# MIT-SPARK/TEASER-plusplus

Hardware: AMD Instinct MI355X
Metric: registrations/sec at N=10000 correspondences, 95% outliers (higher is better)
Workload: dtype bf16x3-split MFMA + f32 filter with FP64 fix-up for K1 (bitmap bit-identical to FP64); f64 estimators

## Files before the change

include/teaser_hip.h:

```cpp
#ifndef TEASER_HIP_H_
#define TEASER_HIP_H_

#include <stddef.h>
#include <stdint.h>

#ifdef __cplusplus
extern "C" {
#endif

#define TEASER_HIP_ABI_VERSION 1

#if defined(__GNUC__)
#define TEASER_HIP_API __attribute__((visibility("default")))
#else
#define TEASER_HIP_API
#endif

typedef enum teaser_hip_status {
  TEASER_HIP_OK = 0,
  TEASER_HIP_ERR_BAD_ARG = 1,
  TEASER_HIP_ERR_HIP = 2,
  TEASER_HIP_ERR_NO_DEVICE = 3,
  TEASER_HIP_ERR_UNSUPPORTED = 4,
  TEASER_HIP_ERR_TIME_LIMIT = 5,
// ... 101 lines not shown
TEASER_HIP_API int32_t teaser_hip_multi_create(const teaser_params_c* params, const int32_t* devices,
                                int32_t n_devices , teaser_hip_multi** out);
TEASER_HIP_API int32_t teaser_hip_multi_destroy(teaser_hip_multi* mh);
TEASER_HIP_API int32_t teaser_hip_multi_solve_batch(teaser_hip_multi* mh, const double* const* src,
                                     const double* const* dst, const int32_t* n, int32_t batch,
                                     teaser_solution_c* out );
TEASER_HIP_API int32_t teaser_hip_multi_route(teaser_hip_multi* mh, int32_t problem, teaser_hip_solver** h,
                               int32_t* local_problem);
TEASER_HIP_API int32_t teaser_hip_multi_device_count(const teaser_hip_multi* mh);

#define TEASER_HIP_COMM_ID_BYTES 128
typedef struct teaser_hip_comm teaser_hip_comm;
TEASER_HIP_API int32_t teaser_hip_comm_shard(int64_t total, int32_t rank, int32_t world, int64_t* first, int64_t* last);
TEASER_HIP_API int32_t teaser_hip_comm_unique_id(uint8_t* id );
TEASER_HIP_API int32_t teaser_hip_comm_create(const uint8_t* id, int32_t rank, int32_t world, int32_t device,
                               teaser_hip_comm** out);
TEASER_HIP_API int32_t teaser_hip_comm_destroy(teaser_hip_comm* c);
TEASER_HIP_API int32_t teaser_hip_comm_gather_solutions(teaser_hip_comm* c, const teaser_solution_c* local,
                                         int64_t n_local, int64_t total, teaser_solution_c* all );
TEASER_HIP_API int32_t teaser_hip_comm_gather_indices(teaser_hip_comm* c, teaser_hip_solver* h, int64_t n_local,
                                       int64_t total, int32_t k_max, int32_t* lens, int32_t* indices);
TEASER_HIP_API const char* teaser_hip_comm_last_error(const teaser_hip_comm* c);

TEASER_HIP_API int32_t teaser_hip_get_max_clique(teaser_hip_solver* h, int32_t problem, int32_t* buf, int64_t* len);
TEASER_HIP_API int32_t teaser_hip_get_rotation_inliers(teaser_hip_solver* h, int32_t problem, int32_t* buf,
                                        int64_t* len);
TEASER_HIP_API int32_t teaser_hip_get_translation_inliers(teaser_hip_solver* h, int32_t problem, int32_t* buf,
                                           int64_t* len);
TEASER_HIP_API int32_t teaser_hip_get_input_ordered_translation_inliers(teaser_hip_solver* h, int32_t problem,
                                                         int32_t* buf, int64_t* len);
TEASER_HIP_API int32_t teaser_hip_get_inlier_graph_bitmap(teaser_hip_solver* h, int32_t problem, uint64_t* buf,
                                           int64_t* len );
TEASER_HIP_API int32_t teaser_hip_get_degrees(teaser_hip_solver* h, int32_t problem, int32_t* buf, int64_t* len);

TEASER_HIP_API int32_t teaser_hip_solve_for_rotation(teaser_hip_solver* h, const double* src, const double* dst,
                                      int32_t k, double noise_bound, double* rotation_rowmajor,
                                      uint8_t* inlier_mask, double* cost, int32_t* iterations);
TEASER_HIP_API int32_t teaser_hip_solve_for_translation(teaser_hip_solver* h, const double* src,
                                         const double* dst, int32_t k, double* translation,
                                         uint8_t* inlier_mask);
TEASER_HIP_API int32_t teaser_hip_scalar_tls(teaser_hip_solver* h, const double* x, const double* ranges,
                              int32_t n, double* estimate, uint8_t* inlier_mask);
TEASER_HIP_API int32_t teaser_hip_solve_for_scale(teaser_hip_solver* h, const double* v1, const double* v2,
                                   int64_t m, double* scale, uint8_t* inlier_mask);

TEASER_HIP_API int32_t teaser_hip_compute_fpfh(teaser_hip_solver* h, const float* cloud_xyz, int32_t n,
                                double normal_radius, double fpfh_radius, float* fpfh_out,
                                float* normals_out);
TEASER_HIP_API int32_t teaser_hip_match_features(teaser_hip_solver* h, const float* src_feat, int32_t n_src,
                                  const float* dst_feat, int32_t n_dst, int32_t dim, int32_t use_crosscheck,
                                  int32_t* pairs, int64_t* n_pairs);
TEASER_HIP_API int32_t teaser_hip_tuple_test(teaser_hip_solver* h, const float* src_xyz, int32_t n_src,
                              const float* dst_xyz, int32_t n_dst, float tuple_scale, uint64_t seed,
                              int32_t* pairs , int64_t* n_pairs );

typedef struct teaser_certifier_params_c {
  double noise_bound;
  double cbar2;
  double sub_optimality;
  double max_iterations;
  double gamma_tau;
} teaser_certifier_params_c;
typedef struct teaser_certification_c {
  int32_t is_optimal;
  int32_t iterations;
  double best_suboptimality;
// ... 755 lines not shown
```

teaser-plusplus_amd/__init__.py:

```python
import ctypes as C
import enum
import os
import subprocess
import typing

import numpy as np

_HERE = os.path.dirname(os.path.abspath(__file__))
_CSRC = os.path.join(_HERE, "csrc")
LIB_PATH = os.path.join(_HERE, "libteaser_hip.so")

STATUS_NAMES = {0: "OK", 1: "BAD_ARG", 2: "HIP", 3: "NO_DEVICE", 4: "UNSUPPORTED", 5: "TIME_LIMIT",
                6: "SCRATCH", 7: "OOM", 8: "BUSY"}


class TeaserHipError(RuntimeError):
    def __init__(self, status, msg=""):
        self.status = status
        super().__init__("teaser_hip status %d (%s) %s" % (status, STATUS_NAMES.get(status, "?"), msg))


class RotationEstimationAlgorithm(enum.IntEnum):
    GNC_TLS = 0
    FGR = 1
# ... 47 lines not shown
        ("clique_exact_run", C.c_int32),
        ("heuristic_size", C.c_int32),
        ("colour_uncoloured", C.c_int32),
        ("num_edges", C.c_int64),
    ]


class ProfileC(C.Structure):
    _fields_ = [
        ("h2d_ms", C.c_float),
        ("tim_graph_ms", C.c_float),
        ("tim_graph_launches", C.c_int32),
        ("degree_ms", C.c_float),
        ("heuristic_ms", C.c_float),
        ("peel_ms", C.c_float),
        ("exact_ms", C.c_float),
        ("rotation_ms", C.c_float),
        ("translation_ms", C.c_float),
        ("d2h_ms", C.c_float),
        ("total_ms", C.c_float),
        ("tim_graph_pairs", C.c_int64),
        ("tim_graph_bytes", C.c_int64),
        ("colour_ms", C.c_float),
        ("tim_aux_ms", C.c_float),
    ]


EXPORTED_SYMBOLS = [
    "teaser_hip_params_default", "teaser_hip_solver_create", "teaser_hip_solver_destroy",
    "teaser_hip_solver_reset", "teaser_hip_solver_get_params", "teaser_hip_solve",
    "teaser_hip_solve_device", "teaser_hip_solve_correspondences", "teaser_hip_solve_batch",
    "teaser_hip_solve_batch_device", "teaser_hip_get_max_clique", "teaser_hip_get_rotation_inliers",
    "teaser_hip_get_translation_inliers", "teaser_hip_get_input_ordered_translation_inliers",
    "teaser_hip_get_inlier_graph_bitmap", "teaser_hip_get_degrees", "teaser_hip_solve_for_rotation",
    "teaser_hip_solve_for_translation", "teaser_hip_scalar_tls", "teaser_hip_max_clique",
    "teaser_hip_set_profiling", "teaser_hip_set_option", "teaser_hip_get_option", "teaser_hip_get_profile", "teaser_hip_get_stream",
    "teaser_hip_last_error", "teaser_hip_abi_version", "teaser_hip_device_count", "teaser_hip_host_alloc",
    "teaser_hip_host_free",
    "teaser_hip_synth_problem", "teaser_hip_submit_batch", "teaser_hip_wait",
    "teaser_hip_set_pipeline_depth", "teaser_hip_multi_create", "teaser_hip_multi_destroy",
    "teaser_hip_multi_solve_batch", "teaser_hip_multi_route", "teaser_hip_multi_device_count",
    "teaser_hip_solve_for_scale", "teaser_hip_compute_fpfh", "teaser_hip_match_features", "teaser_hip_tuple_test",
    "teaser_hip_certifier_params_default", "teaser_hip_certify", "teaser_hip_certifier_warmup",
    "teaser_hip_certify_dual_projection", "teaser_hip_certify_stages",
    "teaser_hip_comm_shard", "teaser_hip_comm_unique_id", "teaser_hip_comm_create", "teaser_hip_comm_destroy",
    "teaser_hip_comm_gather_solutions", "teaser_hip_comm_gather_indices", "teaser_hip_comm_last_error",
    "teaser_hip_icp_params_default", "teaser_hip_icp_create", "teaser_hip_icp_destroy", "teaser_hip_icp_last_error",
    "teaser_hip_icp_fill_scratch",
    "teaser_hip_icp_batch", "teaser_hip_icp_solve", "teaser_hip_icp_estimation_default", "teaser_hip_icp_batch_ex",
    "teaser_hip_icp_solve_ex", "teaser_hip_icp_batch_cov", "teaser_hip_icp_solve_cov",
    "teaser_hip_icp_covariances_batch", "teaser_hip_icp_normals_batch", "teaser_hip_icp_batch_auto",
    "teaser_hip_icp_solve_auto",
    "teaser_hip_icp_self_knn_batch", "teaser_hip_icp_remove_statistical_outliers_batch",
    "teaser_hip_icp_remove_radius_outliers_batch", "teaser_hip_icp_set_option", "teaser_hip_icp_get_option",
    "teaser_hip_icp_knn_search_batch", "teaser_hip_icp_hybrid_search_batch", "teaser_hip_icp_radius_search_batch",
    "teaser_hip_icp_fpfh_batch", "teaser_hip_icp_boundary_points_batch",
    "teaser_hip_icp_frame_default", "teaser_hip_icp_unproject_depth_batch", "teaser_hip_icp_project_depth_batch",
    "teaser_hip_icp_iss_params_default", "teaser_hip_icp_iss_keypoints_batch",
    "teaser_hip_icp_cluster_dbscan_batch", "teaser_hip_icp_farthest_point_down_sample_batch",
    "teaser_hip_icp_information_batch", "teaser_hip_icp_information",
    "teaser_hip_icp_color_default", "teaser_hip_icp_batch_color", "teaser_hip_icp_solve_color",
    "teaser_hip_icp_color_gradients_batch",
    "teaser_hip_voxel_create", "teaser_hip_voxel_destroy", "teaser_hip_voxel_last_error",
    "teaser_hip_voxel_fill_scratch",
    "teaser_hip_voxel_down_sample_batch", "teaser_hip_voxel_down_sample",
    "teaser_hip_features_create", "teaser_hip_features_destroy", "teaser_hip_features_last_error",
    "teaser_hip_features_fill_scratch",
# ... 45 lines not shown
_vp, _ip, _dp = C.c_void_p, C.POINTER(C.c_int32), C.POINTER(C.c_double)
_u8p, _i64p, _u64p = C.POINTER(C.c_uint8), C.POINTER(C.c_int64), C.POINTER(C.c_uint64)


def lib():
    global _lib
    if _lib is not None:
        return _lib
    if not os.path.exists(LIB_PATH):
        raise ImportError("%s is missing: run __graft_entry__.build() (make -C %s)" % (LIB_PATH, _CSRC))
    os.environ.setdefault("GPU_MAX_HW_QUEUES", "8")
    L = C.CDLL(LIB_PATH)
    L.teaser_hip_host_alloc.argtypes = [C.c_size_t, C.POINTER(_vp)]
    L.teaser_hip_host_free.argtypes = [_vp]
    L.teaser_hip_params_default.argtypes = [C.POINTER(ParamsC)]
    L.teaser_hip_solver_create.argtypes = [C.POINTER(ParamsC), C.c_int32, C.POINTER(_vp)]
    L.teaser_hip_solver_destroy.argtypes = [_vp]
    L.teaser_hip_solver_reset.argtypes = [_vp, C.POINTER(ParamsC)]
    L.teaser_hip_solver_get_params.argtypes = [_vp, C.POINTER(ParamsC)]
    L.teaser_hip_solve.argtypes = [_vp, _dp, _dp, C.c_int32, C.POINTER(SolutionC)]
    L.teaser_hip_solve_device.argtypes = [_vp, _vp, _vp, C.c_int32, C.POINTER(SolutionC)]
    L.teaser_hip_solve_correspondences.argtypes = [_vp, C.POINTER(C.c_float), C.c_int32,
                                                   C.POINTER(C.c_float), C.c_int32, _ip, C.c_int32,
                                                   C.POINTER(SolutionC)]
    L.teaser_hip_solve_batch.argtypes = [_vp, C.POINTER(_dp), C.POINTER(_dp), _ip, C.c_int32,
                                         C.POINTER(SolutionC)]
    L.teaser_hip_solve_batch_device.argtypes = [_vp, _vp, _vp, _i64p, _ip, C.c_int32,
                                                C.POINTER(SolutionC)]
    for nm in ("teaser_hip_get_max_clique", "teaser_hip_get_rotation_inliers",
               "teaser_hip_get_translation_inliers",
               "teaser_hip_get_input_ordered_translation_inliers", "teaser_hip_get_degrees"):
        getattr(L, nm).argtypes = [_vp, C.c_int32, _ip, _i64p]
    L.teaser_hip_get_inlier_graph_bitmap.argtypes = [_vp, C.c_int32, _u64p, _i64p]
    L.teaser_hip_solve_for_rotation.argtypes = [_vp, _dp, _dp, C.c_int32, C.c_double, _dp, _u8p, _dp, _ip]
    L.teaser_hip_solve_for_translation.argtypes = [_vp, _dp, _dp, C.c_int32, _dp, _u8p]
    L.teaser_hip_scalar_tls.argtypes = [_vp, _dp, _dp, C.c_int32, _dp, _u8p]
    L.teaser_hip_solve_for_scale.argtypes = [_vp, _dp, _dp, C.c_int64, _dp, _u8p]
    _fp = C.POINTER(C.c_float)
    L.teaser_hip_compute_fpfh.argtypes = [_vp, _fp, C.c_int32, C.c_double, C.c_double, _fp, _fp]
    L.teaser_hip_match_features.argtypes = [_vp, _fp, C.c_int32, _fp, C.c_int32, C.c_int32, C.c_int32, _ip, _i64p]
    L.teaser_hip_tuple_test.argtypes = [_vp, _fp, C.c_int32, _fp, C.c_int32, C.c_float, C.c_uint64, _ip, _i64p]
    L.teaser_hip_certify.argtypes = [_vp, C.c_void_p, _dp, _dp, _dp, _dp, C.c_int32, C.c_void_p, _dp, C.c_int32]
    L.teaser_hip_certify_dual_projection.argtypes = [_vp, _dp, _dp, C.c_int32, _dp]
    L.teaser_hip_certify_stages.argtypes = [_vp, C.c_void_p, _dp, _dp, _dp, _dp, C.c_int32, C.c_int32, _dp, _dp,
                                            C.c_int32, C.c_void_p]
    L.teaser_hip_max_clique.argtypes = [_vp, _u64p, C.c_int32, _ip, _ip, _ip]
    L.teaser_hip_submit_batch.argtypes = [_vp, _vp, _vp, _i64p, _ip, C.c_int32, C.c_int32, _ip]
    L.teaser_hip_wait.argtypes = [_vp, C.c_int32, C.POINTER(SolutionC)]
    L.teaser_hip_set_pipeline_depth.argtypes = [_vp, C.c_int32]
    L.teaser_hip_multi_create.argtypes = [C.POINTER(ParamsC), _ip, C.c_int32, C.POINTER(_vp)]
    L.teaser_hip_multi_destroy.argtypes = [_vp]
    L.teaser_hip_multi_solve_batch.argtypes = [_vp, C.POINTER(_dp), C.POINTER(_dp), _ip, C.c_int32,
                                               C.POINTER(SolutionC)]
    L.teaser_hip_multi_route.argtypes = [_vp, C.c_int32, C.POINTER(_vp), _ip]
    L.teaser_hip_multi_device_count.argtypes = [_vp]
    L.teaser_hip_set_profiling.argtypes = [_vp, C.c_int32]
    L.teaser_hip_set_option.argtypes = [_vp, C.c_char_p, C.c_int64]
    L.teaser_hip_get_option.argtypes = [C.c_char_p, C.POINTER(C.c_int64)]
    L.teaser_hip_get_profile.argtypes = [_vp, C.POINTER(ProfileC)]
    L.teaser_hip_get_stream.argtypes = [_vp]
    L.teaser_hip_get_stream.restype = _vp
    L.teaser_hip_last_error.argtypes = [_vp]
    L.teaser_hip_last_error.restype = C.c_char_p
    L.teaser_hip_synth_problem.argtypes = [C.c_uint64, C.c_int32, C.c_double, C.c_double, _dp, _dp,
                                           _dp, _dp, _u8p]
    from . import icp as _icp
# ... 904 lines not shown
```

teaser-plusplus_amd/csrc/internal.h:

```cpp
#pragma once

#include <hip/hip_runtime.h>
#include <stdint.h>

#include <atomic>
#include <mutex>
#include <algorithm>
#include <vector>

#include "teaser_hip.h"

namespace thip {

constexpr int kWave = 64;
constexpr int kMaxStarts = 16;
constexpr int kPeelRounds = 3;
constexpr int kSmallCap = 768;

struct ProbDesc {
  int32_t n;
  int32_t W;
  int64_t pt_off;
  int64_t bm_off;
  int64_t w_off;
};

#ifndef TEASER_TAIL_PRIO
#define TEASER_TAIL_PRIO 3
#endif
#define TAIL_WAVE_PRIO() __builtin_amdgcn_s_setprio(TEASER_TAIL_PRIO)

struct ProbState {
  int32_t lb;
  int32_t best_start;
  int32_t alive_count;
  int32_t peel_done;
  int32_t proven;
  int32_t clique_size;
  int32_t n_rot;
  int32_t n_trans;
  int32_t gnc_iters;
  int32_t x_count;
  int32_t k1_overflow;
  int32_t max_core;
  int32_t tls_arrive;
  int32_t heu_closed;
  int32_t next_start;
  int32_t scale_overflow;
  int32_t deg_closed;
  int32_t heu_best;
  int32_t start_vertex[kMaxStarts];
  int32_t start_size[kMaxStarts];
  unsigned long long deg_sum;
  double scale;
  double R[9];
  double t[3];
  double gnc_cost;
};
// ... 234 lines not shown
```

teaser-plusplus_amd/csrc/kernels_clique.hip:

```cpp
#include <algorithm>
#include <utility>

#include <mutex>

#include "internal.h"

namespace thip {

struct LevelHdr {
  int32_t pcount;
  int32_t m;
  int32_t idx;
  int32_t pad;
  int64_t prev_off;
  int64_t bytes;
};

__device__ __forceinline__ int64_t align16(int64_t x) { return (x + 15) & ~(int64_t)15; }

__device__ __forceinline__ int wsum(int v) {
#pragma unroll
  for (int o = 32; o > 0; o >>= 1) v += __shfl_xor(v, o, 64);
  return v;
}
// ... 861 lines not shown
  __syncthreads();
  bool use_x = xc > 0 && xc <= kExactXCap;
  if (xc > 0) {
    for (int k = tid; k < xc; k += 256) {
      const bool ok = xc > kRootPruneCap || keep[d.pt_off + k] >= lb;
      if (ok) {
        const int x = xlist[d.pt_off + k];
        atomicOr(reinterpret_cast<unsigned long long*>(&Xb[x >> 6]), 1ull << (x & 63));
        atomicAdd(&kept, 1);
      }
    }
  }
  __syncthreads();
  const int nx = kept;
  if (xc > 0 && xc <= kRootPruneCap && nx == 0) {
    if (tid == 0) {
      pb->prob = p;
      pb->n2 = 0;
      pb->W2 = 0;
      pb->n_roots = 0;
      pb->use_x = 0;
      pb->lb = lb;
      pb->max_deg = 0;
      pb->ctrl[5] = xc;
      pb->ctrl[6] = 0;
    }
    return;
  }
  if (use_x && nx > 0) {
    const int lane = tid & 63, wave = tid >> 6;
    for (int k = wave; k < xc; k += 4) {
      const int x = xlist[d.pt_off + k];
      if (!((Xb[x >> 6] >> (x & 63)) & 1ull)) continue;
      const uint64_t* row = bm + (int64_t)x * W;
      for (int w = lane; w < W; w += 64) {
        const uint64_t v = row[w] & al[w];
        if (v) atomicOr(reinterpret_cast<unsigned long long*>(&Cb[w]), v);
      }
    }
    __syncthreads();
    for (int w = tid; w < W; w += 256) Cb[w] &= ~Xb[w];
  } else {
    for (int w = tid; w < W; w += 256) {
      Cb[w] = al[w];
      Xb[w] = 0;
    }
    use_x = false;
  }
  __syncthreads();
  int cnt = 0, mdeg = 0;
  for (int w = tid; w < W; w += 256) {
    uint64_t bits = Cb[w] | Xb[w];
    cnt += __popcll(bits);
    cand_bits[d.w_off + w] = Cb[w];
    x_bits[d.w_off + w] = Xb[w];
    while (bits) {
      mdeg = max(mdeg, deg[d.pt_off + w * 64 + __builtin_ctzll(bits)]);
      bits &= bits - 1;
    }
  }
  for (int o = 32; o > 0; o >>= 1) {
    cnt += __shfl_xor(cnt, o, 64);
    mdeg = max(mdeg, __shfl_xor(mdeg, o, 64));
  }
  if ((tid & 63) == 0) red4[tid >> 6] = cnt;
  __syncthreads();
  const int n2 = red4[0] + red4[1] + red4[2] + red4[3];
// ... 85 lines not shown
__global__ __launch_bounds__(256) void exact_rank_kernel(const ExactProb* __restrict__ probs,
                                                         const unsigned long long* __restrict__ key_pool,
                                                         int32_t* __restrict__ order_pool) {
  __shared__ unsigned long long tile[256];
  const ExactProb pb = probs[blockIdx.y];
  const int nx = pb.use_x ? pb.n_roots : 0, m = pb.n2 - nx;
  if (pb.n2 <= 0 || (int)blockIdx.x * 256 >= m) return;
  const unsigned long long* keys = key_pool + pb.order_off + nx;
  const int i = blockIdx.x * 256 + threadIdx.x;
  const unsigned long long mine = i < m ? keys[i] : ~0ull;
  int rank = 0;
  for (int base = 0; base < m; base += 256) {
    __syncthreads();
    tile[threadIdx.x] = base + (int)threadIdx.x < m ? keys[base + threadIdx.x] : ~0ull;
    __syncthreads();
    const int lim = min(256, m - base);
    for (int k = 0; k < lim; ++k) rank += tile[k] < mine ? 1 : 0;
  }
  if (i < m) order_pool[pb.order_off + nx + rank] = (int32_t)(mine & 0xffffffffu);
}

__global__ __launch_bounds__(256) void exact_gather_kernel(const ProbDesc* __restrict__ descs,
                                                           const ExactProb* __restrict__ probs,
                                                           const uint64_t* __restrict__ bitmap,
                                                           const int32_t* __restrict__ order_pool,
                                                           uint64_t* __restrict__ bitmap_pool) {
  const ExactProb pb = probs[blockIdx.y];
  const int lane = threadIdx.x & 63, wave = threadIdx.x >> 6;
  const int n2 = pb.n2, W2 = pb.W2;
  const ProbDesc d = descs[pb.prob];
  const int32_t* order = order_pool + pb.order_off;
  uint64_t* out = bitmap_pool + pb.bm_off;
  for (int i = blockIdx.x * 4 + wave; i < n2; i += gridDim.x * 4) {
    const uint64_t* row = bitmap + d.bm_off + (int64_t)order[i] * d.W;
    for (int wo = 0; wo < W2; ++wo) {
      const int j = wo * 64 + lane;
      bool e = false;
      if (j < n2) {
        const int v = order[j];
        e = (row[v >> 6] >> (v & 63)) & 1ull;
      }
      const uint64_t m = __ballot(e);
      if (lane == 0) out[(int64_t)i * W2 + wo] = m;
    }
  }
}

void launch_exact_build(hipStream_t s, const ProbDesc* d_desc, const ExactProb* d_probs, int nprob, int max_W,
                        int max_n2, const uint64_t* d_bitmap, const int32_t* d_deg, const uint64_t* d_cand_bits,
                        const uint64_t* d_x_bits, int32_t* d_order_pool, unsigned long long* d_key_pool,
                        uint64_t* d_bitmap_pool) {
  if (nprob <= 0 || max_n2 <= 0) return;
  hipLaunchKernelGGL(exact_list_kernel, dim3(nprob), dim3(256), 0, s, d_desc, d_probs, d_deg, d_cand_bits, d_x_bits,
                     d_order_pool, d_key_pool);
  hipLaunchKernelGGL(exact_rank_kernel, dim3((max_n2 + 255) / 256, nprob), dim3(256), 0, s, d_probs, d_key_pool,
                     d_order_pool);
  hipLaunchKernelGGL(exact_gather_kernel, dim3(std::min((max_n2 + 3) / 4, 2048), nprob), dim3(256), 0, s, d_desc,
                     d_probs, d_bitmap, d_order_pool, d_bitmap_pool);
}

__global__ __launch_bounds__(256) void exact_finish_kernel(const ProbDesc* __restrict__ descs,
                                                           const ExactProb* __restrict__ probs,
                                                           const int32_t* __restrict__ order_pool,
                                                           const int32_t* __restrict__ clique_pool,
                                                           int32_t* __restrict__ clique,
                                                           ProbState* __restrict__ states) {
  extern __shared__ __attribute__((aligned(16))) char smem[];
// ... 174 lines not shown
}

constexpr int kColourWaves = 16, kAssignWaves = 16;

__global__ __launch_bounds__(64 * kAssignWaves) void colour_assign_kernel(const ProbDesc* __restrict__ descs,
                                                            const int32_t* __restrict__ sel,
                                                            const uint64_t* __restrict__ bitmap,
                                                            ProbState* __restrict__ states,
                                                            int32_t* __restrict__ colour,
                                                            int32_t* __restrict__ tent,
                                                            const int32_t* __restrict__ list,
                                                            const int32_t* __restrict__ counts,
                                                            int32_t* __restrict__ xlist,
                                                            const uint64_t* __restrict__ colbits, int round,
                                                            int count_idx, const uint64_t* __restrict__ alive,
                                                            uint64_t* __restrict__ bid_snapshot) {
  __shared__ unsigned long long Fs[kAssignWaves][kColourMaxWords];
  const int p = sel ? sel[blockIdx.y] : (int)blockIdx.y;
  const ProbDesc d = descs[p];
  if (!sel && colour_not_needed(states[p], d.n)) return;
  const int lane = threadIdx.x & 63, wave = threadIdx.x >> 6;
  if (bid_snapshot && blockIdx.x == 0)
    for (int w = threadIdx.x; w < d.W; w += 64 * kAssignWaves) bid_snapshot[d.w_off + w] = alive[d.w_off + w] & ~colbits[d.w_off + w];
  const int count = counts[(int64_t)blockIdx.y * (kColourRounds + 2) + count_idx];
  int32_t* col = colour + d.pt_off;
  const int lb = states[p].lb;
  const int nw = (lb + 63) >> 6;
  unsigned long long* F = Fs[wave];
  const uint64_t* cb = colbits + d.w_off;
  for (int it = blockIdx.x * kAssignWaves + wave; it < count; it += gridDim.x * kAssignWaves) {
    const int v = list[d.pt_off + it];
    F[lane] = 0ull;
    __builtin_amdgcn_fence(__ATOMIC_ACQ_REL, "wavefront");
    const uint64_t* row = bitmap + d.bm_off + (int64_t)v * d.W;
    for (int w0 = 0; w0 < d.W; w0 += 64 * kRowWordsPerLane) {
      uint64_t words[kRowWordsPerLane];
#pragma unroll
      for (int k = 0; k < kRowWordsPerLane; ++k) {
        const int w = w0 + 64 * k + lane;
        words[k] = w < d.W ? (row[w] & cb[w]) : 0ull;
      }
      visit_bits_batched(words, w0, lane, [&](int u) { return col[u]; },
                         [&](int, int cu) {
                           if (cu >= 0) atomicOr(&F[cu >> 6], 1ull << (cu & 63));
                         });
    }
    __builtin_amdgcn_fence(__ATOMIC_ACQ_REL, "wavefront");
    unsigned long long freeb = 0ull;
    if (lane < nw) {
      freeb = ~F[lane];
      const int rem = lb - lane * 64;
      if (rem < 64) freeb &= (1ull << rem) - 1ull;
    }
    const int cnt = __popcll(freeb);
    int incl = cnt;
#pragma unroll
    for (int o = 1; o < 64; o <<= 1) {
      const int t = __shfl_up(incl, o, 64);
      if (lane >= o) incl += t;
    }
    const int total = __shfl(incl, 63, 64);
    if (total == 0) {
      if (lane == 0) {
        col[v] = -2;
        tent[d.pt_off + v] = -1;
        xlist[d.pt_off + atomicAdd(&states[p].x_count, 1)] = v;
      }
// ... 11 lines not shown
}

__global__ __launch_bounds__(64 * kColourWaves) void colour_resolve_kernel(const ProbDesc* __restrict__ descs,
                                                             const int32_t* __restrict__ sel,
                                                             const uint64_t* __restrict__ bitmap,
                                                             ProbState* __restrict__ states,
                                                             int32_t* __restrict__ colour,
                                                             const int32_t* __restrict__ tent,
                                                             const int32_t* __restrict__ list,
                                                             int32_t* __restrict__ next_list,
                                                             int32_t* __restrict__ counts,
                                                             int32_t* __restrict__ xlist,
                                                             uint64_t* __restrict__ colbits,
                                                             const uint64_t* __restrict__ bidders ,
                                                             int round, int last, int count_idx, int next_idx) {
  __shared__ int lostv[kColourWaves];
  const int p = sel ? sel[blockIdx.y] : (int)blockIdx.y;
  const ProbDesc d = descs[p];
  if (!sel && colour_not_needed(states[p], d.n)) return;
  const int lane = threadIdx.x & 63, wave = threadIdx.x >> 6;
  int32_t* cnt = counts + (int64_t)blockIdx.y * (kColourRounds + 2);
  const int count = cnt[count_idx];
  int32_t* col = colour + d.pt_off;
  const int32_t* tn = tent + d.pt_off;
  const uint64_t* bd = bidders + d.w_off;
  for (int it0 = blockIdx.x * kColourWaves; it0 < count; it0 += gridDim.x * kColourWaves) {
    const int it = it0 + wave;
    const int v = it < count ? list[d.pt_off + it] : -1;
    const bool consider = v >= 0 && col[v] == -1;
    bool lose = false;
    if (consider) {
      const int tv = tn[v];
      const unsigned int pv = colour_hash(v, round, 0xabcdef1u);
      const uint64_t* row = bitmap + d.bm_off + (int64_t)v * d.W;
      for (int w0 = 0; w0 < d.W; w0 += 64 * kRowWordsPerLane) {
        uint64_t words[kRowWordsPerLane];
#pragma unroll
        for (int k = 0; k < kRowWordsPerLane; ++k) {
          const int w = w0 + 64 * k + lane;
          words[k] = w < d.W ? (row[w] & bd[w]) : 0ull;
        }
        visit_bits_batched(words, w0, lane, [&](int u) { return tn[u]; },
                           [&](int u, int tu) {
                             if (tu == tv) {
                               const unsigned int pu = colour_hash(u, round, 0xabcdef1u);
                               lose |= (pu > pv) | ((pu == pv) & (u > v));
                             }
                           });
      }
      const bool lost = __ballot(lose) != 0ull;
      if (lane == 0) {
        if (!lost) {
          col[v] = tv;
          atomicOr(reinterpret_cast<unsigned long long*>(colbits + d.w_off + (v >> 6)), 1ull << (v & 63));
        }
        lostv[wave] = lost ? v : -1;
      }
    } else if (lane == 0) {
      lostv[wave] = -1;
    }
    __syncthreads();
    if (wave == 0) {
      const int x = lane < kColourWaves ? lostv[lane] : -1;
      const uint64_t m = __ballot(x >= 0);
      if (m) {
        int base = 0;
        if (lane == 0) base = atomicAdd(last ? &states[p].x_count : &cnt[next_idx], __builtin_popcountll(m));
// ... 97 lines not shown
    tab[v] = c >= 0 ? (unsigned short)c : kPcNone;
  }
  for (int w = tid; w < d.W; w += kPcThreads) {
    cbm[w] = colbits[d.w_off + w];
    bdm[w] = 0ull;
  }
  __syncthreads();
  auto stamp = [&](int r, int k) {
    if (dbg && blockIdx.x == 0 && blockIdx.y == 0 && tid == 0) dbg[r * 16 + k] = (long long)wall_clock64();
  };
  for (int r = 0; r < rounds; ++r) {
    const bool cls = r < kColourClasses;
    const int j = r - kColourClasses;
    const int32_t* cur = (cls ? class_lists + (int64_t)r * total_n : ((j & 1) ? list_b : list_a)) + d.pt_off;
    int32_t* nxt = (cls ? list_a : ((j & 1) ? list_a : list_b)) + d.pt_off;
    const int count_idx = cls ? r : kColourClasses + j;
    const int next_idx = cls ? kColourClasses : kColourClasses + j + 1;
    const bool last = r == rounds - 1;
    const int count = cnt[count_idx];
    if (count == 0) {
      if (cls) continue;
      break;
    }
    stamp(r, 0);
    for (int it = blockIdx.x * kPcWaves + wave; it < count; it += nwg * kPcWaves) {
      const int v = cur[it];
      const bool probe = dbg && it == 0;
      if (probe) {
        asm volatile("" :: "v"(v));
        stamp(r, 8);
      }
      F[lane] = 0ull;
      __builtin_amdgcn_fence(__ATOMIC_ACQ_REL, "wavefront");
      const uint64_t* row = bitmap + d.bm_off + (int64_t)v * d.W;
      for (int w0 = 0; w0 < d.W; w0 += 64 * kRowWordsPerLane) {
        uint64_t words[kRowWordsPerLane];
#pragma unroll
        for (int k = 0; k < kRowWordsPerLane; ++k) {
          const int w = w0 + 64 * k + lane;
          words[k] = w < d.W ? (row[w] & cbm[w]) : 0ull;
        }
        if (probe && w0 == 0) {
          asm volatile("s_waitcnt vmcnt(0)" ::: "memory");
          stamp(r, 9);
        }
        pc_visit<kPcFly>(words, w0, lane, tab, [&](int, unsigned int t) {
          if (t < 0x8000u) atomicOr(&F[t >> 6], 1ull << (t & 63));
        });
      }
      __builtin_amdgcn_fence(__ATOMIC_ACQ_REL, "wavefront");
      if (probe) stamp(r, 10);
      unsigned long long freeb = 0ull;
      if (lane < nw) {
        freeb = ~F[lane];
        const int rem = lb - lane * 64;
        if (rem < 64) freeb &= (1ull << rem) - 1ull;
      }
      const int fc = __popcll(freeb);
      int incl = fc;
#pragma unroll
      for (int o = 1; o < 64; o <<= 1) {
        const int t = __shfl_up(incl, o, 64);
        if (lane >= o) incl += t;
      }
      const int total = __shfl(incl, 63, 64);
      if (total == 0) {
        if (lane == 0) {
// ... 12 lines not shown
        lg[it] = lane * 64 + __builtin_ctzll(b);
      }
      if (probe) stamp(r, 11);
    }
    __syncthreads();
    stamp(r, 1);
    if (!pc_grid_sync(sync, nwg, target, &sh_flag)) return;
    stamp(r, 2);
    for (int it0 = 0; it0 < count; it0 += 8 * kPcThreads) {
      int c[8], v[8];
#pragma unroll
      for (int q = 0; q < 8; ++q) {
        const int it = it0 + q * kPcThreads + tid;
        c[q] = it < count ? lg[it] : -1;
        v[q] = it < count ? cur[it] : 0;
      }
#pragma unroll
      for (int q = 0; q < 8; ++q)
        if (c[q] >= 0) {
          tab[v[q]] = (unsigned short)(0x8000 | c[q]);
          atomicOr(&bdm[v[q] >> 6], 1ull << (v[q] & 63));
        }
    }
    __syncthreads();
    stamp(r, 3);
    for (int it0 = blockIdx.x * kPcWaves; it0 < count; it0 += nwg * kPcWaves) {
      const int it = it0 + wave;
      const int v = it < count ? cur[it] : -1;
      const int tv = v >= 0 ? lg[it] : -1;
      bool lose = false;
      if (tv >= 0) {
        const unsigned int mine = 0x8000u | (unsigned int)tv;
        const unsigned int pv = colour_hash(v, r, 0xabcdef1u);
        const uint64_t* row = bitmap + d.bm_off + (int64_t)v * d.W;
        for (int w0 = 0; w0 < d.W; w0 += 64 * kRowWordsPerLane) {
          uint64_t words[kRowWordsPerLane];
#pragma unroll
          for (int k = 0; k < kRowWordsPerLane; ++k) {
            const int w = w0 + 64 * k + lane;
            words[k] = w < d.W ? (row[w] & bdm[w]) : 0ull;
          }
          pc_visit<kPcFly>(words, w0, lane, tab, [&](int u, unsigned int t) {
            if (t == mine) {
              const unsigned int pu = colour_hash(u, r, 0xabcdef1u);
              lose |= (pu > pv) | ((pu == pv) & (u > v));
            }
          });
        }
        const bool lost = __ballot(lose) != 0ull;
        if (lane == 0) {
          if (!lost) {
            col[v] = tv;
            lg[it] = tv | 0x40000000;
            atomicOr(reinterpret_cast<unsigned long long*>(colbits + d.w_off + (v >> 6)), 1ull << (v & 63));
          }
          lostv[wave] = lost ? v : -1;
        }
      } else if (lane == 0) {
        lostv[wave] = -1;
      }
      __syncthreads();
      if (wave == 0) {
        const int x = lane < kPcWaves ? lostv[lane] : -1;
        const uint64_t m = __ballot(x >= 0);
        if (m) {
          int base = 0;
          if (lane == 0) base = atomicAdd(last ? &states[p].x_count : &cnt[next_idx], __builtin_popcountll(m));
// ... 50 lines not shown
                                                            const ProbState* __restrict__ states,
                                                            int32_t* __restrict__ tent) {
  const int p = sel ? sel[blockIdx.y] : (int)blockIdx.y;
  const ProbDesc d = descs[p];
  if (!sel && colour_not_needed(states[p], d.n)) return;
  const int xc = min(states[p].x_count, kRootPruneCap);
  for (int i = blockIdx.x * 256 + threadIdx.x; i < xc; i += gridDim.x * 256) tent[d.pt_off + i] = 0;
}



__global__ __launch_bounds__(256) void root_prune_kernel(const ProbDesc* __restrict__ descs,
                                                         const int32_t* __restrict__ sel,
                                                         const uint64_t* __restrict__ bitmap,
                                                         const uint64_t* __restrict__ alive,
                                                         const ProbState* __restrict__ states,
                                                         const int32_t* __restrict__ xlist,
                                                         int32_t* __restrict__ count) {
  extern __shared__ __attribute__((aligned(16))) char smem[];
  __shared__ int wsum_[4];
  const int p = sel ? sel[blockIdx.z] : (int)blockIdx.z;
  const ProbDesc d = descs[p];
  if (!sel && colour_not_needed(states[p], d.n)) return;
  const int xc = states[p].x_count;
  if (xc > kRootPruneCap) return;
  const int lb = states[p].lb;
  uint64_t* Rx = reinterpret_cast<uint64_t*>(smem);
  const uint64_t* bm = bitmap + d.bm_off;
  const uint64_t* al = alive + d.w_off;
  const int lane = threadIdx.x & 63, wave = threadIdx.x >> 6;
  for (int root = blockIdx.y; root < xc; root += gridDim.y) {
  const int x = xlist[d.pt_off + root];
  __syncthreads();
  for (int w = threadIdx.x; w < d.W; w += 256) Rx[w] = bm[(int64_t)x * d.W + w] & al[w];
  __syncthreads();
  int cnt = 0;
  for (int w = blockIdx.x * 4 + wave; w < d.W; w += 4 * gridDim.x) {
    uint64_t bits = Rx[w];
    while (bits) {
      const int y0 = w * 64 + __builtin_ctzll(bits);
      bits &= bits - 1;
      const bool two = bits != 0ull;
      const int y1 = two ? w * 64 + __builtin_ctzll(bits) : y0;
      bits &= bits - (two ? 1ull : 0ull);
      const uint64_t* r0 = bm + (int64_t)y0 * d.W;
      const uint64_t* r1 = bm + (int64_t)y1 * d.W;
      int c0 = 0, c1 = 0;
      for (int k0 = 0; k0 < d.W; k0 += 64 * 8) {
        uint64_t a[8], b[8];
#pragma unroll
        for (int j = 0; j < 8; ++j) {
          const int k = k0 + 64 * j + lane;
          a[j] = k < d.W ? r0[k] : 0ull;
          b[j] = (two && k < d.W) ? r1[k] : 0ull;
        }
#pragma unroll
        for (int j = 0; j < 8; ++j) {
          const int k = k0 + 64 * j + lane;
          const uint64_t m = k < d.W ? Rx[k] : 0ull;
          c0 += __popcll(a[j] & m);
          c1 += __popcll(b[j] & m);
        }
      }
      c0 = wsum(c0);
      c1 = wsum(c1);
      cnt += (c0 >= lb - 1) ? 1 : 0;
      cnt += (two && c1 >= lb - 1) ? 1 : 0;
    }
  }
  if (lane == 0) wsum_[wave] = cnt;
  __syncthreads();
  if (threadIdx.x == 0) {
    const int t = wsum_[0] + wsum_[1] + wsum_[2] + wsum_[3];
    if (t) atomicAdd(&count[d.pt_off + root], t);
  }
  }
}

constexpr int kMisBidders = 256;
// ... 69 lines not shown
  const int p = sel ? sel[blockIdx.y] : (int)blockIdx.y;
  const ProbDesc d = descs[p];
  if (!sel && colour_not_needed(states[p], d.n)) return;
  const int lb = states[p].lb, lbc = min(lb, mb.cap);
  const int lane = threadIdx.x & 63;
  if (blockIdx.x == 0 && threadIdx.x == 0) states[p].x_count = 0;
  const int32_t* cl = clique + d.pt_off;
  const int npad = d.W * 64;
  int mine = 0;
  for (int v0 = blockIdx.x * 256; v0 < npad; v0 += gridDim.x * 256) {
    const int v = v0 + threadIdx.x;
    const bool in = v < d.n;
    const bool al = in && ((alive[d.w_off + (v >> 6)] >> (v & 63)) & 1ull);
    int c = al ? -1 : -3;
    if (al) {
      int lo = 0, hi = lb;
      while (lo < hi) {
        const int mid = (lo + hi) >> 1;
        if (cl[mid] < v) lo = mid + 1; else hi = mid;
      }
      if (lo < lb && cl[lo] == v) c = lo;
    }
    if (in) colour[d.pt_off + v] = c;
    const uint64_t m = __ballot(c == -1);
    if (lane == 0 && v < npad) {
      unc[d.w_off + (v >> 6)] = m;
      mine += __builtin_popcountll(m);
    }
  }
  if (mine) atomicAdd(&mb.ucount[4 * blockIdx.y], mine);
  uint64_t* nc = mb.nc + (size_t)blockIdx.y * mb.cap * mb.max_W;
  const uint64_t* bm = bitmap + d.bm_off;
  for (int c = blockIdx.x; c < lbc; c += gridDim.x) {
    const uint64_t* row = bm + (int64_t)cl[c] * d.W;
    for (int w = threadIdx.x; w < d.W; w += 256) nc[(size_t)c * mb.max_W + w] = row[w];
  }
}

__device__ __forceinline__ int mis_admit_k(int uncoloured, int lbc) {
  const int k = (uncoloured + 128 * lbc - 1) / (128 * lbc);
  return k < 1 ? 1 : k;
}

constexpr int kMisSlab = 4;
constexpr int kMisSlabPitch = kMisSlab + 1;
__global__ __launch_bounds__(256) void mis_bid_kernel(const ProbDesc* __restrict__ descs, const int32_t* __restrict__ sel,
                                                      const ProbState* __restrict__ states, const uint64_t* __restrict__ unc,
                                                      MisBuf mb, int round) {
  extern __shared__ __attribute__((aligned(16))) char smem[];
  uint64_t* slab = reinterpret_cast<uint64_t*>(smem);
  __shared__ uint64_t ubs[kMisSlab];
  const int p = sel ? sel[blockIdx.y] : (int)blockIdx.y;
  const ProbDesc d = descs[p];
  if (!sel && colour_not_needed(states[p], d.n)) return;
  const int lane = threadIdx.x & 63, wave = threadIdx.x >> 6;
  const int j0 = blockIdx.x * kMisSlab;
  if (j0 >= d.W) return;
  const int uc = mb.ucount[4 * blockIdx.y];
  const int lbc = min(states[p].lb, mb.cap);
  const int K = mis_admit_k(uc, lbc);
  if (threadIdx.x < kMisSlab) {
    const int j = j0 + threadIdx.x;
    ubs[threadIdx.x] = j < d.W ? unc[d.w_off + j] : 0ull;
  }
  __syncthreads();
  uint64_t any = 0ull;
#pragma unroll
// ... 136 lines not shown
  }
  __syncthreads();
  const int my_u = t < cnt ? sorted[t] : 0;
  bool pending = t < cnt;
  int nwon = 0;
  for (;;) {
    const bool elig = pending && !((ncl[my_u >> 6] >> (my_u & 63)) & 1ull);
    pending = elig;
    const uint64_t bal = __ballot(elig);
    if (lane == 0) wmask[wave] = bal;
    if (t < kMisBatch) adjm[t] = 0ull;
    __syncthreads();
    int before = __builtin_popcountll(bal & ((1ull << lane) - 1ull)), total = 0;
#pragma unroll
    for (int w2 = 0; w2 < 4; ++w2) {
      const int pc = __builtin_popcountll(wmask[w2]);
      before += w2 < wave ? pc : 0;
      total += pc;
    }
    if (total == 0) break;
    const int ncand = total < kMisBatch ? total : kMisBatch;
    int mycand = -1;
    if (elig && before < kMisBatch) {
      cand[before] = my_u;
      mycand = before;
      pending = false;
    }
    __syncthreads();
    {
      constexpr int kTpc = kMisBidders / kMisBatch, kPpt = kMisBatch / kTpc, kGrp = kPpt < 8 ? kPpt : 8;
      static_assert(kMisBatch <= 64 && kTpc * kPpt == kMisBatch && kPpt % kGrp == 0, "thread mapping of the adjacency gather");
      const int a = t / kTpc;
      const int ua = a < ncand ? cand[a] : 0;
      const uint64_t* rowa = bm + (int64_t)ua * W;
      unsigned long long bits = 0ull;
#pragma unroll
      for (int g0 = 0; g0 < kPpt; g0 += kGrp) {
        uint64_t wd[kGrp];
        int ubv[kGrp];
#pragma unroll
        for (int q = 0; q < kGrp; ++q) {
          const int b = (t % kTpc) * kPpt + g0 + q;
          const bool on = a < ncand && b < a;
          ubv[q] = on ? cand[b] : -1;
          wd[q] = on ? rowa[ubv[q] >> 6] : 0ull;
        }
#pragma unroll
        for (int q = 0; q < kGrp; ++q)
          if (ubv[q] >= 0 && ((wd[q] >> (ubv[q] & 63)) & 1ull)) bits |= 1ull << ((t % kTpc) * kPpt + g0 + q);
      }
      if (bits) atomicOr(&adjm[a], bits);
    }
    __syncthreads();
    unsigned long long acc = 0ull;
    {
      const unsigned long long mine = lane < kMisBatch ? adjm[lane] : 0ull;
      const unsigned int mlo = (unsigned int)mine, mhi = (unsigned int)(mine >> 32);
      for (int a = 0; a < ncand; ++a) {
        const unsigned long long ma = ((unsigned long long)(unsigned int)__builtin_amdgcn_readlane((int)mhi, a) << 32) |
                                      (unsigned int)__builtin_amdgcn_readlane((int)mlo, a);
        if ((ma & acc) == 0ull) acc |= 1ull << a;
      }
    }
    unsigned long long todo = acc;
    while (todo) {
      constexpr int kFly = 8;
      const uint64_t* rows[kFly];
#pragma unroll
      for (int q = 0; q < kFly; ++q) {
        if (todo) {
          rows[q] = bm + (int64_t)cand[__builtin_ctzll(todo)] * W;
          todo &= todo - 1ull;
        } else {
          rows[q] = nullptr;
        }
      }
      uint64_t got[kFly][4];
#pragma unroll
      for (int q = 0; q < kFly; ++q)
#pragma unroll
        for (int m = 0; m < 4; ++m) {
          const int w = t + 256 * m;
          got[q][m] = (rows[q] && w < W) ? rows[q][w] : 0ull;
        }
#pragma unroll
      for (int q = 0; q < kFly; ++q)
#pragma unroll
        for (int m = 0; m < 4; ++m) nc[m] |= got[q][m];
    }
#pragma unroll
    for (int m = 0; m < 4; ++m) {
      const int w = t + 256 * m;
      if (w < W) ncl[w] = nc[m];
    }
    if (mycand >= 0 && ((acc >> mycand) & 1ull)) {
      colour[d.pt_off + my_u] = c;
      atomicAnd(reinterpret_cast<unsigned long long*>(unc + d.w_off + (my_u >> 6)), ~(1ull << (my_u & 63)));
      ++nwon;
    }
    __syncthreads();
  }
  if (nwon) atomicAdd(&won_total, nwon);
#pragma unroll
  for (int m = 0; m < 4; ++m) {
// ... 8 lines not shown
  }
}

__global__ __launch_bounds__(256) void mis_finish_kernel(const ProbDesc* __restrict__ descs, const int32_t* __restrict__ sel,
                                                         ProbState* __restrict__ states, const uint64_t* __restrict__ unc,
                                                         int32_t* __restrict__ colour, int32_t* __restrict__ xlist) {
  const int p = sel ? sel[blockIdx.y] : (int)blockIdx.y;
  const ProbDesc d = descs[p];
  if (!sel && colour_not_needed(states[p], d.n)) return;
  for (int w = blockIdx.x * 256 + threadIdx.x; w < d.W; w += gridDim.x * 256) {
    uint64_t bits = unc[d.w_off + w];
    if (!bits) continue;
    int base = atomicAdd(&states[p].x_count, __builtin_popcountll(bits));
    while (bits) {
      const int v = w * 64 + __builtin_ctzll(bits);
      bits &= bits - 1;
      colour[d.pt_off + v] = -2;
      xlist[d.pt_off + base++] = v;
    }
  }
}

__global__ __launch_bounds__(256) void mis_verify_kernel(const ProbDesc* __restrict__ descs, const int32_t* __restrict__ sel,
                                                         const uint64_t* __restrict__ bitmap, const int32_t* __restrict__ colour,
                                                         int* __restrict__ out ) {
  const int p = sel ? sel[blockIdx.y] : (int)blockIdx.y;
  const ProbDesc d = descs[p];
  const int lane = threadIdx.x & 63;
  const int32_t* col = colour + d.pt_off;
  for (int v = blockIdx.x * 4 + (threadIdx.x >> 6); v < d.n; v += gridDim.x * 4) {
    const int cv = col[v];
    if (cv < 0) continue;
    int bad = 0;
    const uint64_t* row = bitmap + d.bm_off + (int64_t)v * d.W;
    for (int w = lane; w < d.W; w += 64) {
      uint64_t bits = row[w];
      while (bits) {
        const int u = w * 64 + __builtin_ctzll(bits);
        bits &= bits - 1;
        bad += (u < d.n && col[u] == cv) ? 1 : 0;
      }
    }
    bad = wsum(bad);
    if (lane == 0) {
      if (bad) atomicAdd(&out[2 * blockIdx.y], bad);
      atomicAdd(&out[2 * blockIdx.y + 1], 1);
    }
  }
}

namespace {
struct ColourPersistentGate {
  static std::mutex& mu() {
    static std::mutex m;
    return m;
  }
  static hipEvent_t& event_of(int dev) {
    static hipEvent_t ev[64] = {};
    return ev[dev & 63];
  }
  hipStream_t s;
  int dev = 0;
  explicit ColourPersistentGate(hipStream_t stream) : s(stream) {
    mu().lock();
    (void)hipGetDevice(&dev);
    hipEvent_t& e = event_of(dev);
    if (e) (void)hipStreamWaitEvent(s, e, 0);
// ... 184 lines not shown
    __syncthreads();
    if (lane == 0) red[wave] = cnt;
    __syncthreads();
    int total = 0;
    for (int q = 0; q < kCoreWaves; ++q) total += red[q];
    __syncthreads();
    if (total == 0) {
      if (lane == 0) red[wave] = mind;
      __syncthreads();
      int m = 0x7fffffff;
      for (int q = 0; q < kCoreWaves; ++q) m = min(m, red[q]);
      __syncthreads();
      k = m;
      continue;
    }
    max_core = k;
    remaining -= total;
    for (int w = tid; w < W; w += kCoreThreads) {
      uint64_t f = front[w];
      alive[w] &= ~f;
      while (f) {
        cr[w * 64 + __builtin_ctzll(f)] = k;
        f &= f - 1;
      }
    }
    __syncthreads();
    int ord = 0;
    for (int w = 0; w < W; ++w) {
      uint64_t f = front[w];
      while (f) {
        const int b = __builtin_ctzll(f);
        f &= f - 1;
        if ((ord++ & (kCoreWaves - 1)) != wave) continue;
        const uint64_t* row = bm + (int64_t)(w * 64 + b) * W;
        for (int x = lane; x < W; x += 64) {
          uint64_t m = row[x] & alive[x];
          while (m) {
            __hip_atomic_fetch_add(&rd[x * 64 + __builtin_ctzll(m)], -1, __ATOMIC_RELAXED, __HIP_MEMORY_SCOPE_AGENT);
            m &= m - 1;
          }
        }
      }
    }
    __syncthreads();
  }
  ProbState* st = states + blockIdx.x;
  if (tid == 0) st->max_core = max_core;
  if (!(threshold != 1.0 && max_core > (int)(threshold * (double)n))) return;
  for (int w = wave; w < W; w += kCoreWaves) {
    const int v = w * 64 + lane;
    const uint64_t f = __ballot(v < n && cr[v] >= max_core);
    if (lane == 0) {
      front[w] = f;
      wcnt[w] = __builtin_popcountll(f);
    }
  }
  __syncthreads();
  if (tid == 0) {
    int acc = 0;
    for (int w = 0; w < W; ++w) {
      const int c = wcnt[w];
      wcnt[w] = acc;
      acc += c;
    }
    st->clique_size = acc;
    st->lb = acc;
    st->proven = 1;
// ... 23 lines not shown
```

teaser-plusplus_amd/csrc/kernels_graph.hip:

```cpp
#include <algorithm>
#include <utility>
#include <vector>

#include <cstdio>
#include <cstdlib>

#include "internal.h"
#include "fixup_item.h"
#include "fixup_regions.h"
#include "k1_consts.h"
#include "wave_utils.h"

namespace thip {

struct EdgeConst {
  double beta;
  double beta2;
  double m2beta2;
  double beta4;
  double s_hat;
};

__device__ __forceinline__ bool tim_edge_exact(double ax, double ay, double az, double bx,
                                               double by, double bz, double beta) {
// ... 70 lines not shown
      e = tim_edge_scaled(sjx - six, sjy - siy, sjz - siz, djx - dix, djy - diy, djz - diz, kc);
      m = __builtin_amdgcn_ballot_w64(e);
    }
    if (B < 32) {
      own_lo |= e ? (1u << (B & 31)) : 0u;
      asm volatile("" : "+v"(own_lo));
    } else {
      own_hi |= e ? (1u << (B & 31)) : 0u;
      asm volatile("" : "+v"(own_hi));
    }
    asm volatile("v_writelane_b32 %0, %1, %2" : "+v"(tr_lo) : "s"((int)(unsigned int)m), "n"(B));
    asm volatile("v_writelane_b32 %0, %1, %2" : "+v"(tr_hi) : "s"((int)(unsigned int)(m >> 32)), "n"(B));
  }
  template <int... Bs>
  __device__ __forceinline__ void run(const EdgeConst& kc, std::integer_sequence<int, Bs...>) {
    (step<Bs>(kc), ...);
  }
};

__device__ __forceinline__ void tim_block_coords(int gx, int gy, int* I, int* X) {
  const int nblk = gx * gy;
  const int pid = blockIdx.x;
  int lid = pid;
  if (pid < (nblk & ~127)) lid = (pid & ~127) | ((pid & 7) << 4) | ((pid >> 3) & 15);
  *I = lid % gy;
  *X = lid / gy;
}

template <int MODE>
__device__ __forceinline__ void tim_wave_fp64(const double* __restrict__ ps,
                                              const double* __restrict__ pd,
                                              uint64_t* __restrict__ bm, int n, int W, int I,
                                              int Jbase, const EdgeConst& kc, double* cbw) {
  const int T = W;
  const int lane = threadIdx.x & 63;
  const int i = I * 64 + lane;
  const bool vi = i < n;
  const int ic = vi ? i : n - 1;
  const double six = ps[3 * ic], siy = ps[3 * ic + 1], siz = ps[3 * ic + 2];
  const double dix = pd[3 * ic], diy = pd[3 * ic + 1], diz = pd[3 * ic + 2];
  const uint64_t rowmask = (n - I * 64 >= 64) ? ~0ull : ((1ull << (n - I * 64)) - 1ull);

  for (int s = 0; s < kColTilesPerWave; ++s) {
    const int J = Jbase + s;
    if (J < I || J >= T) continue;
    const int j0 = J * 64;
    {
      const int jc = min(j0 + lane, n - 1);
      double* w = cbw + 6 * lane;
      w[0] = ps[3 * jc]; w[1] = ps[3 * jc + 1]; w[2] = ps[3 * jc + 2];
      w[3] = pd[3 * jc]; w[4] = pd[3 * jc + 1]; w[5] = pd[3 * jc + 2];
    }
    ColTile<MODE> ct;
    ct.cb = cbw;
    ct.six = six; ct.siy = siy; ct.siz = siz; ct.dix = dix; ct.diy = diy; ct.diz = diz;
    ct.own_lo = 0; ct.own_hi = 0; ct.tr_lo = 0; ct.tr_hi = 0; ct.unc_cols = 0;
    ct.cb_addr = (int)(uintptr_t)cbw;
    asm volatile("" ::: "memory");
    ct.template load_col<0>(ct.pf[0]);
    ct.template load_col<1>(ct.pf[1]);
    ct.template load_col<2>(ct.pf[2]);
    ct.run(kc, std::make_integer_sequence<int, 64>());
    uint64_t own = ((uint64_t)ct.own_hi << 32) | ct.own_lo;
    uint64_t trw = ((uint64_t)(unsigned int)ct.tr_hi << 32) | (unsigned int)ct.tr_lo;
    if (MODE == 0) {
      uint64_t todo = ct.unc_cols;
      while (todo) {
        const int b = __builtin_ctzll(todo);
        todo &= todo - 1;
        const int jc = min(j0 + b, n - 1);
        const bool e = tim_edge_exact(ps[3 * jc] - six, ps[3 * jc + 1] - siy, ps[3 * jc + 2] - siz,
                                      pd[3 * jc] - dix, pd[3 * jc + 1] - diy, pd[3 * jc + 2] - diz,
                                      kc.beta);
        const uint64_t m = __ballot(e);
        own = (own & ~(1ull << b)) | ((uint64_t)(e ? 1 : 0) << b);
        trw = (lane == b) ? m : trw;
      }
    }
    const uint64_t colmask = (n - j0 >= 64) ? ~0ull : ((1ull << (n - j0)) - 1ull);
    own &= colmask;
    if (J == I) own &= ~(1ull << lane);
    if (vi) bm[(int64_t)i * W + J] = own;
    if (J != I && j0 + lane < n) {
      bm[(int64_t)(j0 + lane) * W + I] = trw & rowmask;
    }
  }
}

template <int MODE>
__global__ __launch_bounds__(256) void tim_graph_kernel(const ProbDesc* __restrict__ descs,
                                                        const double* __restrict__ src,
                                                        const double* __restrict__ dst,
                                                        uint64_t* __restrict__ bitmap,
                                                        double beta, int gx, int gy,
                                                        const ProbState* __restrict__ states) {
  const ProbDesc d = descs[blockIdx.y];
  const int n = d.n, W = d.W;
  const int T = W;
  int I, X;
  tim_block_coords(gx, gy, &I, &X);
  if (I >= T) return;
  const int wave = __builtin_amdgcn_readfirstlane(threadIdx.x >> 6);
  const int Jbase = (X * kWavesPerBlock + wave) * kColTilesPerWave;
  if (Jbase + kColTilesPerWave - 1 < I || Jbase >= T) return;

  __shared__ __attribute__((aligned(16))) double cbuf[kWavesPerBlock][64 * 6];
  EdgeConst kc;
  kc.beta = beta;
  kc.beta2 = beta * beta;
  kc.m2beta2 = -2.0 * kc.beta2;
  kc.beta4 = kc.beta2 * kc.beta2;
  kc.s_hat = 1.0;
  if (MODE == 1) kc.s_hat = states[blockIdx.y].scale;
  tim_wave_fp64<MODE>(src + 3 * d.pt_off, dst + 3 * d.pt_off, bitmap + d.bm_off, n, W, I, Jbase, kc,
                      cbuf[wave]);
}

typedef float f32x16 __attribute__((ext_vector_type(16)));
// ... 258 lines not shown
}
#endif

__global__ void tim_prep_consts_kernel(TimPrep* __restrict__ prep, int batch, double beta) {
  const int p = blockIdx.x * blockDim.x + threadIdx.x;
  if (p >= batch) return;
  const k1c::ConstsXY c = k1c::consts_xy(beta, k1c::norm_shift(prep_half_extent(prep + p)), prep[p].r2_bits);
  prep[p].band_c = c.C;
  prep[p].use_mfma = c.use_mfma;
}
#ifdef TEASER_K1_LAB
__global__ void tim_prep_consts3_kernel(TimPrep* __restrict__ prep, int batch, double beta) {
  const int p = blockIdx.x * blockDim.x + threadIdx.x;
  if (p >= batch) return;
  const k1c::Consts c = k1c::consts(beta, k1c::norm_shift(prep_half_extent(prep + p)), prep[p].r2_bits);
  prep[p].band_c = c.C;
  prep[p].use_mfma = c.use_mfma;
}
#endif


constexpr bool kK1Pipe = false, kK1Plain = true;
constexpr int kK1Chunks = 1, kK1Occ = 3;

template <bool PIPE, bool PLAIN, int OCC, int CHUNKS, bool LOWER, bool UW3 = false>
__global__ __launch_bounds__(256, OCC) void tim_graph_mfma3_kernel(
    const ProbDesc* __restrict__ descs, const double* __restrict__ src,
    const double* __restrict__ dst, const void* __restrict__ ops, const TimPrep* __restrict__ prep,
    uint64_t* __restrict__ bitmap, double beta, int gyr,
    unsigned long long* __restrict__ work, unsigned int* __restrict__ work_count,
    ProbState* __restrict__ states, int32_t* __restrict__ deg, unsigned long long* __restrict__ regions, int Tmax) {
  const ProbDesc d = descs[blockIdx.y];
  const int n = d.n, W = d.W;
  const int T = W;
  int Ig, X;
  fxr::decode_block((int)blockIdx.x, (int)gridDim.x, gyr, CHUNKS, &Ig, &X);
  constexpr int kBlockColTiles = kMfmaColTiles * CHUNKS;
  const int I0 = Ig * kMfmaRowTiles, Jbase = X * kBlockColTiles;
  auto region_of = [&](int wv, int chunk) -> unsigned long long* {
    const int Iw = I0 + wv, Xc = X * CHUNKS + chunk;
    return fxr::is_cell(Iw, Xc, Tmax) ? regions + fxr::region_offset((int)blockIdx.y, Tmax, Iw, Xc) : nullptr;
  };
  auto zero_regions = [&]() {
    if ((threadIdx.x & 63) < CHUNKS) {
      unsigned long long* r = region_of((int)(threadIdx.x >> 6), (int)(threadIdx.x & 63));
      if (r) r[0] = 0ull;
    }
  };
  if (I0 >= T || Jbase >= T || Jbase + kBlockColTiles - 1 < I0) {
    zero_regions();
    return;
  }
  const int lane = threadIdx.x & 63;
  const int wave = __builtin_amdgcn_readfirstlane(threadIdx.x >> 6);
  const int I = I0 + wave;

  const double* __restrict__ ps = src + 3 * d.pt_off;
  const double* __restrict__ pd = dst + 3 * d.pt_off;
  uint64_t* __restrict__ bm = bitmap + d.bm_off;
  __shared__ __attribute__((aligned(16))) uint64_t lds_own[kMfmaRowTiles][64][kMfmaColTiles + 1];
  static_assert(sizeof(lds_own[0]) >= sizeof(double) * 64 * 6 && sizeof(lds_own[0]) >= 8 * kWorkBuf, "aliased buffers");
  __shared__ __attribute__((aligned(16))) uint64_t lds_tr[kMfmaColTiles][64][kMfmaRowTiles];
  constexpr int kRowOps = UW3 ? 3 : kTimRowOperands;
  constexpr int kTileBytes = 2 * (kRowOps + kTimColOperands) * 1024, kColBase = 2 * kRowOps * 1024;
  static_assert(UW3 || (kTileBytes == (int)sizeof(TimOperandTile2) && kColBase == (int)offsetof(TimOperandTile2, b)), "tile layout");
  const char* __restrict__ qt = reinterpret_cast<const char*>(ops) + (size_t)d.w_off * kTileBytes;
  const int h = lane >> 5, c = lane & 31;
// ... 9 lines not shown
  {
    const int It = min(I, T - 1);
    for (int rt = 0; rt < 2; ++rt)
      for (int m = 0; m < kRowOps; ++m) ar[rt][m] = __builtin_bit_cast(f16x8, load_op(It, 0, rt, m));
  }
  const bool rowvalid = I < T;
  const uint64_t rowmask = !rowvalid ? 0ull : (n - I * 64 >= 64) ? ~0ull : ((1ull << (n - I * 64)) - 1ull);
  const int Jfirst = max(Jbase, I), Jend = min(Jbase + kBlockColTiles, T);
  uint4 bX[kTimColOperands], bY[kTimColOperands];
  {
    const int Jf = min(Jfirst, T - 1);
    for (int m = 0; m < kTimColOperands; ++m) bX[m] = load_op(Jf, 1, 0, m);
    if (PIPE)
      for (int m = 0; m < kTimColOperands; ++m) bY[m] = load_op(Jf, 1, 1, m);
  }
  const TimPrep pr = prep[blockIdx.y];
  if (!pr.use_mfma) {
    EdgeConst kc;
    kc.beta = beta;
    kc.beta2 = beta * beta;
    kc.m2beta2 = -2.0 * kc.beta2;
    kc.beta4 = kc.beta2 * kc.beta2;
    kc.s_hat = 1.0;
    if (I < T)
      for (int jb = Jbase; jb < Jbase + kBlockColTiles; jb += kColTilesPerWave)
        if (!(jb + kColTilesPerWave - 1 < I || jb >= T))
          tim_wave_fp64<0>(ps, pd, bm, n, W, I, jb, kc, reinterpret_cast<double*>(&lds_own[wave][0][0]));
    zero_regions();
    return;
  }
  const __amdgpu_buffer_rsrc_t deg_rsrc = __builtin_amdgcn_make_buffer_rsrc(
      (void*)(deg + d.pt_off), 0, (int)((unsigned int)n * 4u), 0x00020000);
  const __amdgpu_buffer_rsrc_t bm_rsrc = __builtin_amdgcn_make_buffer_rsrc(
      (void*)bm, 0, (int)((unsigned int)n * (unsigned int)W * 8u), 0x00020000);
  int degacc = 0;
  const int cq = c - 4 * h;
  const int selfq = (cq >= 0 && (cq & 4) == 0) ? ((cq & 3) | ((cq >> 3) << 2)) : -1;
  unsigned int flags = 0;
  const float thr = pr.band_c;

  struct Acc {
    f32x16 U, W;
  };
  static_assert(!(UW3 && PIPE), "the three-MFMA lab variant has the flat schedule only");
  auto mf = [&](Acc& a, const f16x8(&arow)[kRowOps], const uint4(&b)[kTimColOperands]) {
    f32x16 z;
    for (int k = 0; k < 16; ++k) z[k] = 0.f;
    a.W = __builtin_amdgcn_mfma_f32_32x32x16_f16(arow[0], __builtin_bit_cast(f16x8, b[0]), z, 0, 0, 0);
    a.U = __builtin_amdgcn_mfma_f32_32x32x16_f16(arow[1], __builtin_bit_cast(f16x8, b[1]), a.W, 0, 0, 0);
  };
  auto epi = [&](const Acc& a, bool self_tile) -> unsigned int {
    unsigned int colbits = 0;
    float m = INFINITY;
#pragma unroll
    for (int qp = 7; qp >= 0; --qp) {
      float d0, d1;
      if (PLAIN) {
        d0 = __builtin_fmaf(a.U[2 * qp], a.U[2 * qp], a.W[2 * qp]);
        d1 = __builtin_fmaf(a.U[2 * qp + 1], a.U[2 * qp + 1], a.W[2 * qp + 1]);
      } else {
        const f32x2 u2 = {a.U[2 * qp], a.U[2 * qp + 1]}, w2 = {a.W[2 * qp], a.W[2 * qp + 1]};
        const f32x2 d2 = __builtin_elementwise_fma(u2, u2, w2);
        d0 = d2.x;
        d1 = d2.y;
      }
      float v0 = __builtin_fabsf(d0), v1 = __builtin_fabsf(d1);
      if (self_tile) {
// ... 145 lines not shown
    const int Ja = rowvalid ? max(Jc0, Jfirst) : Jc1;
    if (Ja < Jc1) {
      int J = Ja;
      if (PIPE) {
        if (!primed) {
          mf(accA, ar[0], bX);
          __builtin_amdgcn_sched_barrier(0);
          primed = true;
        }
        if (J == I) {
          body_pipe(J, std::true_type());
          ++J;
        }
#pragma nounroll
        for (; J < Jc1; ++J) body_pipe(J, std::false_type());
      } else {
        if (J == I) {
          body_flat(J, std::true_type());
          ++J;
        }
#pragma nounroll
        for (; J < Jc1; ++J) body_flat(J, std::false_type());
      }
    }
    const int nact = max(Jc1 - Ja, 0);
    {
      __syncthreads();
#pragma unroll
      for (int it = 0; it < (kMfmaColTiles * 64) / 256; ++it) {
        const int idx = it * 256 + (int)threadIdx.x, Jr = idx >> 6, r = idx & 63, J = Jc0 + Jr, j = J * 64 + r;
        const uint4 lo = *reinterpret_cast<const uint4*>(&lds_tr[Jr][r][0]);
        const uint4 hi = *reinterpret_cast<const uint4*>(&lds_tr[Jr][r][2]);
        const bool rowok = J < Jc1 && j < n;
        const unsigned int base = ((unsigned int)j * (unsigned int)W + (unsigned int)I0) * 8u;
        if (Jc0 > I0 + 3 && I0 + 3 < T) {
          const int cnt = (__builtin_popcount(lo.x) + __builtin_popcount(lo.y)) + (__builtin_popcount(lo.z) + __builtin_popcount(lo.w)) +
                          (__builtin_popcount(hi.x) + __builtin_popcount(hi.y)) + (__builtin_popcount(hi.z) + __builtin_popcount(hi.w));
          if (LOWER) {
            __builtin_amdgcn_raw_buffer_store_b128(u32x4{lo.x, lo.y, lo.z, lo.w}, bm_rsrc, rowok ? base : kOobOffset, 0, 0);
            __builtin_amdgcn_raw_buffer_store_b128(u32x4{hi.x, hi.y, hi.z, hi.w}, bm_rsrc, rowok ? base + 16u : kOobOffset, 0, 0);
          }
          __builtin_amdgcn_raw_ptr_buffer_atomic_add_i32(cnt, deg_rsrc, (rowok && cnt) ? (unsigned int)j * 4u : kOobOffset, 0, 0);
          continue;
        }
        bool ok[4];
        for (int k = 0; k < 4; ++k) ok[k] = rowok && I0 + k < T && I0 + k < J;
        const unsigned int w32[8] = {lo.x, lo.y, lo.z, lo.w, hi.x, hi.y, hi.z, hi.w};
        int cnt = 0;
        for (int k = 0; k < 4; ++k) cnt += ok[k] ? __builtin_popcount(w32[2 * k]) + __builtin_popcount(w32[2 * k + 1]) : 0;
        if (!LOWER) {
        } else if (ok[3]) {
          __builtin_amdgcn_raw_buffer_store_b128(u32x4{lo.x, lo.y, lo.z, lo.w}, bm_rsrc, base, 0, 0);
          __builtin_amdgcn_raw_buffer_store_b128(u32x4{hi.x, hi.y, hi.z, hi.w}, bm_rsrc, base + 16u, 0, 0);
        } else {
          for (int k = 0; k < 3; ++k)
            __builtin_amdgcn_raw_buffer_store_b64(u32x2{w32[2 * k], w32[2 * k + 1]}, bm_rsrc,
                                                  ok[k] ? base + 8u * k : kOobOffset, 0, 0);
        }
        __builtin_amdgcn_raw_ptr_buffer_atomic_add_i32(cnt, deg_rsrc, cnt ? (unsigned int)j * 4u : kOobOffset, 0, 0);
      }
      if (CHUNKS > 1) __syncthreads();
    }
    if (nact > 0) {
      const int kk = lane & 7, J = Jc0 + kk;
      const bool colok = J >= Ja && J < Jc1;
      const unsigned int off0 = ((unsigned int)(I * 64 + (lane >> 3)) * (unsigned int)W + (unsigned int)J) * 8u;
#pragma unroll
      for (int it = 0; it < 8; ++it) {
        const int r = it * 8 + (lane >> 3);
        const uint64_t w = lds_own[wave][r][kk];
        __builtin_amdgcn_raw_buffer_store_b64(u32x2{(unsigned int)w, (unsigned int)(w >> 32)}, bm_rsrc,
                                              (colok && I * 64 + r < n) ? off0 + (unsigned int)it * 64u * (unsigned int)W : kOobOffset,
                                              0, 0);
      }
    }
    int wcount = 0;
    {
      unsigned int vf = flags;
      if (I * 64 + 4 * h >= n) vf &= ~0xAAAAAAAAu;
      if (I * 64 + 32 + 4 * h >= n) vf &= ~0x55555555u;
      if (T - 1 >= Ja && T - 1 < Jc1 && (n & 63)) {
        const int sh = 4 * (Jc1 - T);
        if ((T - 1) * 64 + c >= n) vf &= ~(0xCu << sh);
        if ((T - 1) * 64 + 32 + c >= n) vf &= ~(0x3u << sh);
      }
      if (__builtin_amdgcn_ballot_w64(vf != 0u) != 0ull) {
        const int mine = __builtin_popcount(vf);
        int base = 0, total = 0;
#pragma unroll
        for (int bit = 0; bit < 6; ++bit) {
          const uint64_t m = __builtin_amdgcn_ballot_w64(((mine >> bit) & 1) != 0);
          base += (int)__builtin_amdgcn_mbcnt_hi((unsigned int)(m >> 32), __builtin_amdgcn_mbcnt_lo((unsigned int)m, 0u)) << bit;
          total += __builtin_popcountll(m) << bit;
        }
        if (total > kWorkBuf) {
          if (lane == 0) states[blockIdx.y].k1_overflow = 1;
        } else {
          int kk = base;
#pragma nounroll
          while (vf) {
            const int pos = 31 - __builtin_clz(vf);
            vf &= ~(1u << pos);
            const int J = Ja + (nact - 1 - (pos >> 2));
            const int ct = ((pos >> 1) & 1) ^ 1, rt = (pos & 1) ^ 1;
            const unsigned int rowp = (unsigned int)(I * 64 + 32 * rt + 4 * h);
// ... 16 lines not shown
        if (lane == 0) base = atomicAdd(work_count + blockIdx.y, (unsigned int)extra);
        base = __builtin_amdgcn_readfirstlane(base);
        if (base + (unsigned int)extra > pr.seg_cap) {
          if (lane == 0) states[blockIdx.y].k1_overflow = 1;
        } else {
          unsigned long long* seg = work + (((size_t)pr.seg_off_hi << 32) | (size_t)pr.seg_off_lo);
#pragma nounroll
          for (int k2i = lane; k2i < extra; k2i += 64) seg[base + k2i] = wbuf[nreg + k2i];
        }
      }
    }
  }
  if (rowvalid)
    __builtin_amdgcn_raw_ptr_buffer_atomic_add_i32(degacc, deg_rsrc, (unsigned int)(I * 64 + lane) * 4u, 0, 0);
}

__global__ __launch_bounds__(256) void tim_fixup_group_kernel(const ProbDesc* __restrict__ descs, int batch,
                                                              const double* __restrict__ src,
                                                              const double* __restrict__ dst,
                                                              uint64_t* __restrict__ bitmap, double beta,
                                                              const unsigned long long* __restrict__ work,
                                                              const unsigned int* __restrict__ work_count,
                                                              ProbState* __restrict__ states,
                                                              int32_t* __restrict__ deg,
                                                              const unsigned long long* __restrict__ regions,
                                                              int Tmax,
                                                              const TimPrep* __restrict__ prep, int upper) {
  TAIL_WAVE_PRIO();
  const int prob = blockIdx.y;
  const unsigned int total = work_count[prob];
  const TimPrep tpr = prep[prob];
  const unsigned int cap = tpr.seg_cap;
  const ProbDesc d = descs[prob];
  const int n = d.n, W = d.W;
  if (total > cap) {
    const int64_t words = (int64_t)n * W;
    uint64_t* bm = bitmap + d.bm_off;
    for (int64_t w = (int64_t)blockIdx.x * 256 + threadIdx.x; w < words; w += (int64_t)gridDim.x * 256) bm[w] = 0;
    if (blockIdx.x == 0 && threadIdx.x == 0) states[prob].k1_overflow = 1;
    return;
  }
  int32_t* dg = deg + d.pt_off;
  if (!tpr.use_mfma) {
    const uint64_t* bm = bitmap + d.bm_off;
    const int lane = threadIdx.x & 63;
    for (int row = blockIdx.x * 4 + (threadIdx.x >> 6); row < n; row += gridDim.x * 4) {
      const uint64_t* r = bm + (int64_t)row * W;
      int c = 0;
      for (int w = lane; w < W; w += 64) c += __popcll(r[w]);
      c = wave_sum_i(c);
      if (lane == 0) dg[row] = c;
    }
    return;
  }
  const double* ps = src + 3 * d.pt_off;
  const double* pd = dst + 3 * d.pt_off;
  unsigned int* bm32 = reinterpret_cast<unsigned int*>(bitmap + d.bm_off);
  EdgeConst kc;
  kc.beta = beta;
  kc.beta2 = beta * beta;
  kc.m2beta2 = -2.0 * kc.beta2;
  kc.beta4 = kc.beta2 * kc.beta2;
  kc.s_hat = 1.0;
  const int lane = threadIdx.x & 63, q = lane & 15, sub = lane >> 4, wave = threadIdx.x >> 6;
  const int rq = (q & 3) + 8 * (q >> 2);
  __shared__ double row_pts[4][64][6];
  __shared__ __attribute__((aligned(16))) double col_pts[4][64][6];
  auto resolve = [&](unsigned long long it, bool valid, auto staged, int tile, int slot) {
    constexpr bool STAGED = decltype(staged)::value;
    int r = fxi::row0(it) + rq, col = fxi::col(it);
    valid = valid && r < n && col < n && r != col;
    r = valid ? r : (STAGED ? tile * 64 : 0);
    col = valid ? col : 0;
    double sx, sy, sz, dx, dy, dz, cx, cy, cz, ex, ey, ez;
    if (STAGED) {
      const double* rp = row_pts[wave][r & 63];
      sx = rp[0]; sy = rp[1]; sz = rp[2]; dx = rp[3]; dy = rp[4]; dz = rp[5];
      const double* cp = col_pts[wave][slot];
      cx = cp[0]; cy = cp[1]; cz = cp[2]; ex = cp[3]; ey = cp[4]; ez = cp[5];
    } else {
      sx = ps[3 * r]; sy = ps[3 * r + 1]; sz = ps[3 * r + 2];
      dx = pd[3 * r]; dy = pd[3 * r + 1]; dz = pd[3 * r + 2];
      cx = ps[3 * col]; cy = ps[3 * col + 1]; cz = ps[3 * col + 2];
      ex = pd[3 * col]; ey = pd[3 * col + 1]; ez = pd[3 * col + 2];
    }
    unsigned int* wp = bm32 + 2 * ((int64_t)r * W + (col >> 6)) + ((col >> 5) & 1);
    const unsigned int bit = 1u << (col & 31);
    bool prov;
    if (STAGED && (r >> 6) != (col >> 6)) {
      prov = fxi::bit(it, q);
    } else {
      prov = (*wp & bit) != 0u;
    }
    const double ax = cx - sx, ay = cy - sy, az = cz - sz, bx = ex - dx, by = ey - dy, bz = ez - dz;
    bool unc, shortp;
    bool e = tim_edge_fast(ax, ay, az, bx, by, bz, kc, &unc, &shortp);
    e |= shortp;
    if (unc) e = tim_edge_exact(ax, ay, az, bx, by, bz, beta);
    if (!valid || prov == e) return;
    atomicXor(wp, bit);
    atomicAdd(dg + r, e ? 1 : -1);
    if ((r >> 6) != (col >> 6)) {
      if (!upper) atomicXor(bm32 + 2 * ((int64_t)col * W + (r >> 6)) + ((r >> 5) & 1), 1u << (r & 31));
      atomicAdd(dg + col, e ? 1 : -1);
    }
  };
  __shared__ unsigned long long queue[4][2 * kRegionWords];
  static_assert(kRegionWords == 64, "one region = one 64-lane load");
  const int T = W, nch = fxr::n_chunks(T);
  auto round = [&](int cnt, int tile) {
    if (lane < cnt) {
      const int col = min(fxi::col(queue[wave][lane]), n - 1);
      double* cp = col_pts[wave][lane];
      const double c0 = ps[3 * col], c1 = ps[3 * col + 1], c2 = ps[3 * col + 2];
      const double e0 = pd[3 * col], e1 = pd[3 * col + 1], e2 = pd[3 * col + 2];
      cp[0] = c0; cp[1] = c1; cp[2] = c2; cp[3] = e0; cp[4] = e1; cp[5] = e2;
    }
    __builtin_amdgcn_fence(__ATOMIC_ACQ_REL, "wavefront");
#pragma nounroll
    for (int base = 0; base < cnt; base += 4) {
      const int k = base + sub;
      resolve(queue[wave][k], k < cnt, std::true_type(), tile, k);
    }
    __builtin_amdgcn_fence(__ATOMIC_ACQ_REL, "wavefront");
  };
  const int wv = blockIdx.x * 4 + wave, nwv = gridDim.x * 4, npairs = (T + 1) >> 1;
  for (int pi = wv; pi < npairs; pi += nwv) {
    for (int side = 0; side < 2; ++side) {
      const int tile = side ? T - 1 - pi : pi;
      if (side && tile == pi) break;
      {
        const int pr = min(tile * 64 + lane, n - 1);
        double* rp = row_pts[wave][lane];
        rp[0] = ps[3 * pr]; rp[1] = ps[3 * pr + 1]; rp[2] = ps[3 * pr + 2];
        rp[3] = pd[3 * pr]; rp[4] = pd[3 * pr + 1]; rp[5] = pd[3 * pr + 2];
      }
// ... 3 lines not shown
      unsigned long long mine = reg[lane];
      for (int Xc = Xc0; Xc < nch; ++Xc) {
        const unsigned long long cur = mine;
        if (Xc + 1 < nch) mine = reg[(size_t)(Xc + 1 - Xc0) * kRegionWords + lane];
        const int cnt = min((int)__builtin_amdgcn_readfirstlane((unsigned int)cur), kRegionItems);
        if (cnt <= 0) continue;
        if (lane >= 1 && lane <= cnt) queue[wave][qn + lane - 1] = cur;
        qn += cnt;
        if (qn >= kRegionWords) {
          __builtin_amdgcn_fence(__ATOMIC_ACQ_REL, "wavefront");
          round(kRegionWords, tile);
          qn -= kRegionWords;
          const unsigned long long moved = queue[wave][kRegionWords + lane];
          __builtin_amdgcn_fence(__ATOMIC_ACQ_REL, "wavefront");
          if (lane < qn) queue[wave][lane] = moved;
        }
      }
      if (qn > 0) {
        __builtin_amdgcn_fence(__ATOMIC_ACQ_REL, "wavefront");
        round(qn, tile);
      }
    }
  }
  const unsigned long long* seg = work + (((size_t)tpr.seg_off_hi << 32) | (size_t)tpr.seg_off_lo);
  const unsigned int ngrp = gridDim.x * 16;
  for (unsigned int w = (blockIdx.x * 256 + threadIdx.x) >> 4; w < total; w += ngrp) resolve(seg[w], true, std::false_type(), 0, 0);
}

constexpr int kMirrorRun = 8;
__global__ __launch_bounds__(256) void tim_mirror_lower_kernel(const ProbDesc* __restrict__ descs,
                                                               uint64_t* __restrict__ bitmap,
                                                               const ProbState* __restrict__ states, int skip_closed) {
  const ProbDesc d = descs[blockIdx.y];
  const int n = d.n, W = d.W, T = W;
  if (T < 2 || (skip_closed && states[blockIdx.y].deg_closed)) return;
  const int lane = threadIdx.x & 63;
  const int runs = (T + kMirrorRun - 1) / kMirrorRun;
  uint64_t* bm = bitmap + d.bm_off;
  for (int wv = blockIdx.x * 4 + (int)(threadIdx.x >> 6); wv < T * runs; wv += gridDim.x * 4) {
    const int J = wv / runs, Ia = (wv % runs) * kMirrorRun, Ib = min(Ia + kMirrorRun, J);
    if (Ia >= Ib) continue;
    uint64_t out[kMirrorRun];
#pragma unroll
    for (int k = 0; k < kMirrorRun; ++k) {
      out[k] = 0ull;
      if (Ia + k >= Ib) continue;
      const uint64_t x = bm[(int64_t)(64 * (Ia + k) + lane) * W + J];
#pragma unroll
      for (int c = 0; c < 64; ++c) {
        const uint64_t m = __builtin_amdgcn_ballot_w64(((x >> c) & 1ull) != 0ull);
        out[k] = lane == c ? m : out[k];
      }
    }
    const int row = 64 * J + lane;
    if (row < n) {
#pragma unroll
      for (int k = 0; k < kMirrorRun; ++k)
        if (Ia + k < Ib) bm[(int64_t)row * W + Ia + k] = out[k];
    }
  }
}

void launch_tim_graph(hipStream_t s, const ProbDesc* d_desc, int batch, int max_n,
                      const double* d_src, const double* d_dst, uint64_t* d_bitmap,
                      double noise_bound, double cbar2, int mode, const ProbState* d_state) {
  if (batch <= 0 || max_n <= 0) return;
  const int T = (max_n + 63) / 64;
  const double beta = 2 * noise_bound * sqrt(cbar2);
  const int gx = (T + kColTilesPerBlock - 1) / kColTilesPerBlock, gy = T;
  dim3 grid(gx * gy, batch);
  if (mode == 0)
    hipLaunchKernelGGL(tim_graph_kernel<0>, grid, dim3(256), 0, s, d_desc, d_src, d_dst, d_bitmap,
                       beta, gx, gy, d_state);
  else
    hipLaunchKernelGGL(tim_graph_kernel<1>, grid, dim3(256), 0, s, d_desc, d_src, d_dst, d_bitmap,
                       beta, gx, gy, d_state);
}

int64_t tim_prep_bytes(int batch) { return (int64_t)batch * ((int64_t)sizeof(TimPrep) + 4) + 64; }
#ifdef TEASER_K1_LAB
int64_t tim_operand_bytes(int64_t total_tiles) { return total_tiles * (int64_t)sizeof(TimOperandTile3); }
#else
int64_t tim_operand_bytes(int64_t total_tiles) { return total_tiles * (int64_t)sizeof(TimOperandTile2); }
#endif

static int tim_mfma_blocks(int T, int chunks) { return fxr::blocks(T, chunks); }
static int64_t tim_region_words(int max_n) { return fxr::arena_words((max_n + 63) / 64); }

static int64_t tim_segment_items(int n) {
  const int64_t seg = std::max<int64_t>((int64_t)n * (n - 1) / 2 / 256, 1 << 16);
  return std::min<int64_t>(seg, 0x7fffffffll);
// ... 114 lines not shown
    } else if (lab.occ4) {
      if (lab.plain) { TIM_K1_LAUNCH_OCC(false, true, 4, 1, true); } else { TIM_K1_LAUNCH_OCC(false, false, 4, 1, true); }
    } else {
      TIM_K1_LAB_CASE(false, false)
      TIM_K1_LAB_CASE(false, true)
      TIM_K1_LAB_CASE(true, false)
      TIM_K1_LAB_CASE(true, true)
    }
#undef TIM_K1_LAB_CASE
#else
    if (upper) {
      TIM_K1_LAUNCH_OCC(kK1Pipe, kK1Plain, kK1Occ, kK1Chunks, false);
    } else {
      TIM_K1_LAUNCH(kK1Pipe, kK1Plain, kK1Chunks);
    }
#endif
#undef TIM_K1_LAUNCH
#undef TIM_K1_LAUNCH_OCC
  } else {
    const int64_t forced_wgs = setting(S_FIXUP_WGS);
    const int64_t fix_wgs = forced_wgs > 0 ? forced_wgs : ((T + 1) / 2 + 3) / 4;
    hipLaunchKernelGGL(tim_fixup_group_kernel, dim3((unsigned)std::max<int64_t>(4, fix_wgs), batch),
                       dim3(256), 0, s, d_desc, batch, d_src, d_dst, d_bitmap, beta, work, work_count, d_state, d_deg,
                       regions, T, prep, upper ? 1 : 0);
  }
}

__global__ __launch_bounds__(256) void degree_kernel(const ProbDesc* __restrict__ descs,
                                                     const uint64_t* __restrict__ bitmap,
                                                     int32_t* __restrict__ deg) {
  const ProbDesc d = descs[blockIdx.y];
  const int lane = threadIdx.x & 63;
  for (int row = blockIdx.x * 4 + (threadIdx.x >> 6); row < d.n; row += gridDim.x * 4) {
    const uint64_t* r = bitmap + d.bm_off + (int64_t)row * d.W;
    int c = 0;
    for (int w = lane; w < d.W; w += 64) c += __popcll(r[w]);
    c = wave_sum_i(c);
    if (lane == 0) deg[d.pt_off + row] = c;
  }
}

void launch_degrees(hipStream_t s, const ProbDesc* d_desc, int batch, int max_n,
                    const uint64_t* d_bitmap, int32_t* d_deg, ProbState* d_state) {
  if (batch <= 0 || max_n <= 0) return;
  dim3 grid((max_n + 3) / 4, batch);
  hipLaunchKernelGGL(degree_kernel, grid, dim3(256), 0, s, d_desc, d_bitmap, d_deg);
}

__global__ __launch_bounds__(256) void trims_kernel(const double* __restrict__ src,
                                                    const double* __restrict__ dst, int n,
                                                    double beta, double* __restrict__ raw,
                                                    double* __restrict__ alpha) {
  const int i = blockIdx.x;
  if (i >= n - 1) return;
  const int64_t seg = (int64_t)i * n - (int64_t)i * (i + 1) / 2;
  const double six = src[3 * i], siy = src[3 * i + 1], siz = src[3 * i + 2];
  const double dix = dst[3 * i], diy = dst[3 * i + 1], diz = dst[3 * i + 2];
  for (int j = i + 1 + threadIdx.x; j < n; j += 256) {
    const double ax = src[3 * j] - six, ay = src[3 * j + 1] - siy, az = src[3 * j + 2] - siz;
    const double bx = dst[3 * j] - dix, by = dst[3 * j + 1] - diy, bz = dst[3 * j + 2] - diz;
    const double v1 = __builtin_sqrt((ax * ax + ay * ay) + az * az);
    const double v2 = __builtin_sqrt((bx * bx + by * by) + bz * bz);
    const int64_t k = seg + (j - i - 1);
    raw[k] = v2 / v1;
    alpha[k] = beta * (1.0 / v1);
  }
}
// ... 33 lines not shown
```

teaser-plusplus_amd/csrc/kernels_heuristic.hip:

```cpp
#include <algorithm>
#include <utility>
#include <vector>

#include <cstdio>
#include <cstdlib>

#include "internal.h"
#include "wave_utils.h"

namespace thip {

constexpr int kGreedyMaxThreads = 512;
constexpr int kCap = 640;
constexpr int kCapW = kCap / 64;
constexpr int kCapStride = kCapW + 1;

template <int kGreedyWaves>
__device__ __forceinline__ int blockN_sum_i(int v, int* red ) {
  v = wave_sum_i(v);
  __syncthreads();
  if ((threadIdx.x & 63) == 0) red[threadIdx.x >> 6] = v;
  __syncthreads();
  int s = 0;
#pragma unroll
  for (int k = 0; k < kGreedyWaves; ++k) s += red[k];
  return s;
}
template <int kGreedyWaves>
__device__ __forceinline__ unsigned long long blockN_max_u64(unsigned long long v,
                                                             unsigned long long* red) {
  v = wave_max_u64(v);
  __syncthreads();
  if ((threadIdx.x & 63) == 0) red[threadIdx.x >> 6] = v;
  __syncthreads();
  unsigned long long m = 0;
#pragma unroll
  for (int k = 0; k < kGreedyWaves; ++k) m = red[k] > m ? red[k] : m;
  return m;
}

template <int kGreedyThreads>
__device__ __forceinline__ int greedy_one_start(
    const ProbDesc* __restrict__ descs, const uint64_t* __restrict__ bitmap,
    const int32_t* __restrict__ deg, ProbState* __restrict__ states,
    int32_t* __restrict__ start_cliques, int64_t total_n, char* smem, const int sidx, long long* trace, const int prob) {
  constexpr int kGreedyWaves = kGreedyThreads / 64;
  long long* tr = trace ? trace + ((size_t)prob * kMaxStarts + sidx) * 8 : nullptr;
  auto stamp = [&](int k) {
    if (tr && threadIdx.x == 0) tr[k] = (long long)wall_clock64();
  };
  auto bump = [&](int k) {
    if (tr && threadIdx.x == 0) tr[k] += 1;
  };
  if (tr && threadIdx.x == 0) tr[6] = tr[7] = 0;
  stamp(0);
  const ProbDesc d = descs[prob];
  const int n = d.n, W = d.W;
  const int Wpad = (W + 1) & ~1;
  uint64_t* P = reinterpret_cast<uint64_t*>(smem);
  uint64_t* U = P + Wpad;
  uint64_t* A = U + Wpad;
  uint64_t* Pc = A + kCap * kCapStride;
  unsigned long long* red64 = reinterpret_cast<unsigned long long*>(Pc + 16);
  int* cand = reinterpret_cast<int*>(red64 + kGreedyMaxThreads / 64);
  int* wcnt = cand + kCap;
  int* red = wcnt + kGreedyMaxThreads;
  int* misc = red + kGreedyMaxThreads / 64;

  ProbState* st = states + prob;
  const int tid = threadIdx.x, lane = tid & 63, wave = tid >> 6;
  const uint64_t* bm = bitmap + d.bm_off;
  const int32_t* dg = deg + d.pt_off;
  int32_t* C = start_cliques + (int64_t)sidx * total_n + d.pt_off;
  int v0 = -1;
  {
    unsigned long long best = 0, sum = 0;
    for (int v = sidx + kMaxStarts * tid; v < n; v += kMaxStarts * kGreedyThreads) {
      const unsigned long long dv = (unsigned int)dg[v];
      const unsigned long long key = ((dv + 1) << 32) | (0xffffffffu - (unsigned int)v);
      best = key > best ? key : best;
    }
    best = blockN_max_u64<kGreedyWaves>(best, red64);
    if (best) v0 = (int)(0xffffffffu - (unsigned int)(best & 0xffffffffu));
    if (sidx == 0) {
      for (int v = tid; v < n; v += kGreedyThreads) sum += (unsigned int)dg[v];
#pragma unroll
      for (int o = 32; o > 0; o >>= 1) sum += __shfl_xor(sum, o, 64);
      __syncthreads();
      if (lane == 0) red64[wave] = sum;
      __syncthreads();
      if (tid == 0) {
        unsigned long long tot = 0;
        for (int k = 0; k < kGreedyWaves; ++k) tot += red64[k];
        st->deg_sum = tot;
      }
      __syncthreads();
    }
    if (tid == 0) st->start_vertex[sidx] = v0;
  }
  if (v0 < 0 || n <= 0) {
    if (threadIdx.x == 0) st->start_size[sidx] = 0;
    return 0;
  }

  int csize = 1;
  if (tid == 0) C[0] = v0;
  int pc = 0;
  for (int w = tid; w < W; w += kGreedyThreads) {
    const uint64_t x = bm[(int64_t)v0 * W + w];
    P[w] = x;
    pc += __popcll(x);
  }
  pc = blockN_sum_i<kGreedyWaves>(pc, red);

  auto cannot_win = [&](int reach) {
    __syncthreads();
    if (tid == 0) misc[1] = __hip_atomic_load(&st->heu_best, __ATOMIC_RELAXED, __HIP_MEMORY_SCOPE_AGENT);
    __syncthreads();
    return reach < misc[1];
  };
  bool gave_up = false;
  stamp(1);
  bool prefer_vote = false;
  while (pc > kCap) {
    if (cannot_win(csize + pc)) {
      gave_up = true;
      pc = 0;
      break;
    }
    bump(prefer_vote ? 7 : 6);
    if (!prefer_vote) {
      unsigned long long key = 0;
      for (int w = tid; w < W; w += kGreedyThreads) {
        uint64_t bits = P[w];
        while (bits) {
          const int u = w * 64 + __builtin_ctzll(bits);
          bits &= bits - 1;
          const unsigned long long k =
              ((unsigned long long)(unsigned int)dg[u] << 32) | (0xffffffffu - (unsigned int)u);
          key = k > key ? k : key;
        }
      }
      key = blockN_max_u64<kGreedyWaves>(key, red64);
      const int u = (int)(0xffffffffu - (unsigned int)(key & 0xffffffffu));
      if (tid == 0) C[csize] = u;
      ++csize;
      int c = 0;
      __syncthreads();
      for (int w = tid; w < W; w += kGreedyThreads) {
        const uint64_t x = P[w] & bm[(int64_t)u * W + w];
        P[w] = x;
        c += __popcll(x);
      }
      c = blockN_sum_i<kGreedyWaves>(c, red);
      prefer_vote = (long long)c * 10 > (long long)pc * 9;
      pc = c;
      continue;
    }
    if (tid == 0) misc[0] = csize;
    unsigned long long bestk = 0;
    const int reach = csize + pc;
    bool hopeless = false;
    constexpr int kListCap = kCap * kCapStride * 2;
    const bool listed = pc <= kListCap;
    if (listed) {
      int* clist = reinterpret_cast<int*>(A);
      {
        const int wpt = (W + kGreedyThreads - 1) / kGreedyThreads;
        const int w0 = tid * wpt, w1 = min(W, w0 + wpt);
        int mycnt = 0;
        for (int w = w0; w < w1; ++w) mycnt += __popcll(P[w]);
        wcnt[tid] = mycnt;
        for (int w = tid; w < W; w += kGreedyThreads) U[w] = 0ull;
        __syncthreads();
        if (wave == 0) {
          constexpr int kPer = kGreedyWaves;
          int a[kPer], tot = 0;
#pragma unroll
          for (int k = 0; k < kPer; ++k) {
            a[k] = wcnt[kPer * lane + k];
            tot += a[k];
          }
          int incl = tot;
// ... 3 lines not shown
            if (lane >= o) incl += t;
          }
          int ex = incl - tot;
#pragma unroll
          for (int k = 0; k < kPer; ++k) {
            wcnt[kPer * lane + k] = ex;
            ex += a[k];
          }
        }
        __syncthreads();
        int pos = wcnt[tid];
        for (int w = w0; w < w1; ++w) {
          uint64_t bits = P[w];
          while (bits) {
            clist[pos++] = w * 64 + __builtin_ctzll(bits);
            bits &= bits - 1;
          }
        }
        __syncthreads();
      }
      constexpr int kStreamRows = kGreedyThreads >= 512 ? 4 : 2;
      for (int i0 = wave * kStreamRows; i0 < pc && !hopeless; i0 += kGreedyWaves * kStreamRows) {
        if (__hip_atomic_load(&st->heu_best, __ATOMIC_RELAXED, __HIP_MEMORY_SCOPE_AGENT) > reach) {
          hopeless = true;
          break;
        }
        int vv[kStreamRows];
        bool on[kStreamRows];
        const uint64_t* rr[kStreamRows];
#pragma unroll
        for (int q = 0; q < kStreamRows; ++q) {
          on[q] = i0 + q < pc;
          vv[q] = clist[on[q] ? i0 + q : i0];
          rr[q] = bm + (int64_t)vv[q] * W;
        }
        int cc[kStreamRows];
#pragma unroll
        for (int q = 0; q < kStreamRows; ++q) cc[q] = 0;
        for (int x0 = 0; x0 < W; x0 += 64 * 8) {
          uint64_t ra[kStreamRows][8];
#pragma unroll
          for (int q = 0; q < kStreamRows; ++q)
#pragma unroll
            for (int j = 0; j < 8; ++j) {
              const int x = x0 + 64 * j + lane;
              ra[q][j] = (on[q] && x < W) ? rr[q][x] : 0ull;
            }
#pragma unroll
          for (int j = 0; j < 8; ++j) {
            const int x = x0 + 64 * j + lane;
            const uint64_t m = x < W ? P[x] : 0ull;
#pragma unroll
            for (int q = 0; q < kStreamRows; ++q) cc[q] += __popcll(ra[q][j] & m);
          }
        }
#pragma unroll
        for (int q = 0; q < kStreamRows; ++q) cc[q] = wave_sum_i(cc[q]);
#pragma unroll
        for (int q = 0; q < kStreamRows; ++q) {
          if (!on[q]) continue;
          if (cc[q] == pc - 1) {
            if (lane == 0) atomicOr(reinterpret_cast<unsigned long long*>(&U[vv[q] >> 6]), 1ull << (vv[q] & 63));
          } else {
            const unsigned long long kk =
                ((unsigned long long)(unsigned int)(cc[q] + 1) << 32) | (0xffffffffu - (unsigned int)vv[q]);
            bestk = kk > bestk ? kk : bestk;
          }
        }
      }
    }
    for (int w = wave; w < W && !hopeless && !listed; w += kGreedyWaves) {
      uint64_t bits = P[w];
      uint64_t uni = 0;
      while (bits) {
        if (__hip_atomic_load(&st->heu_best, __ATOMIC_RELAXED, __HIP_MEMORY_SCOPE_AGENT) > reach) {
          hopeless = true;
          break;
        }
        const int b0 = __builtin_ctzll(bits);
        bits &= bits - 1;
        const bool two = bits != 0ull;
        const int b1 = two ? __builtin_ctzll(bits) : b0;
        bits &= bits - (two ? 1ull : 0ull);
        const uint64_t* r0 = bm + (int64_t)(w * 64 + b0) * W;
        const uint64_t* r1 = bm + (int64_t)(w * 64 + b1) * W;
        int c0 = 0, c1 = 0;
        for (int x0 = 0; x0 < W; x0 += 64 * 8) {
          uint64_t ra[8], rb[8];
#pragma unroll
          for (int j = 0; j < 8; ++j) {
            const int x = x0 + 64 * j + lane;
            ra[j] = x < W ? r0[x] : 0ull;
            rb[j] = (two && x < W) ? r1[x] : 0ull;
          }
#pragma unroll
          for (int j = 0; j < 8; ++j) {
            const int x = x0 + 64 * j + lane;
            const uint64_t m = x < W ? P[x] : 0ull;
            c0 += __popcll(ra[j] & m);
            c1 += __popcll(rb[j] & m);
          }
        }
        c0 = wave_sum_i(c0);
        c1 = wave_sum_i(c1);
#pragma unroll
        for (int k = 0; k < 2; ++k) {
          if (k == 1 && !two) break;
          const int b = k ? b1 : b0, c = k ? c1 : c0;
          if (c == pc - 1) {
            uni |= 1ull << b;
          } else {
            const unsigned long long kk =
                ((unsigned long long)(unsigned int)(c + 1) << 32) | (0xffffffffu - (unsigned int)(w * 64 + b));
            bestk = kk > bestk ? kk : bestk;
          }
        }
      }
      if (lane == 0) U[w] = uni;
    }
    bestk = blockN_max_u64<kGreedyWaves>(bestk, red64);
    if (cannot_win(reach)) {
      gave_up = true;
      pc = 0;
      break;
    }
    int nU = 0;
    for (int w = tid; w < W; w += kGreedyThreads) {
      uint64_t bits = U[w];
      if (bits) {
        const int k = __popcll(bits);
        int pos = atomicAdd(&misc[0], k);
        nU += k;
        P[w] &= ~bits;
        while (bits) {
          C[pos++] = w * 64 + __builtin_ctzll(bits);
          bits &= bits - 1;
        }
      }
    }
    nU = blockN_sum_i<kGreedyWaves>(nU, red);
    csize += nU;
    const int left = pc - nU;
    if (left > 0 && bestk) {
      const int u = (int)(0xffffffffu - (unsigned int)(bestk & 0xffffffffu));
      if (tid == 0) C[csize] = u;
      ++csize;
      int c = 0;
      for (int w = tid; w < W; w += kGreedyThreads) {
        const uint64_t x = P[w] & bm[(int64_t)u * W + w];
        P[w] = x;
        c += __popcll(x);
      }
      c = blockN_sum_i<kGreedyWaves>(c, red);
      prefer_vote = (long long)c * 10 > (long long)left * 9;
      pc = c;
    } else {
      pc = 0;
      __syncthreads();
    }
  }
  stamp(2);
  if (pc > 0) {
    const int wpt = (W + kGreedyThreads - 1) / kGreedyThreads;
    const int w0 = tid * wpt, w1 = min(W, w0 + wpt);
    int mycnt = 0;
    for (int w = w0; w < w1; ++w) mycnt += __popcll(P[w]);
    wcnt[tid] = mycnt;
    __syncthreads();
    if (wave == 0) {
      constexpr int kPer = kGreedyWaves;
      int a[kPer], tot = 0;
#pragma unroll
      for (int k = 0; k < kPer; ++k) {
        a[k] = wcnt[kPer * lane + k];
        tot += a[k];
      }
      int incl = tot;
#pragma unroll
      for (int o = 1; o < 64; o <<= 1) {
        int t = __shfl_up(incl, o, 64);
        if (lane >= o) incl += t;
      }
// ... 7 lines not shown
    __syncthreads();
    {
      int pos = wcnt[tid];
      for (int w = w0; w < w1; ++w) {
        uint64_t bits = P[w];
        while (bits) {
          cand[pos++] = w * 64 + __builtin_ctzll(bits);
          bits &= bits - 1;
        }
      }
    }
    __syncthreads();
    const int Wc = (pc + 63) >> 6;
    int cw[kCapW], cb[kCapW];
    unsigned int vmask = 0;
#pragma unroll
    for (int k = 0; k < kCapW; ++k) {
      const int idx = 64 * k + lane;
      const bool ok = idx < pc;
      const int c = ok ? cand[idx] : 0;
      cw[k] = c >> 5;
      cb[k] = c & 31;
      vmask |= ok ? (1u << k) : 0u;
    }
    const unsigned int* bm32 = reinterpret_cast<const unsigned int*>(bm);
    constexpr int kRowsInFlight = 4;
    for (int r = wave; r < pc; r += kRowsInFlight * kGreedyWaves) {
      const unsigned int* rp[kRowsInFlight];
      bool has[kRowsInFlight];
#pragma unroll
      for (int j = 0; j < kRowsInFlight; ++j) {
        const int rj = r + j * kGreedyWaves;
        has[j] = rj < pc;
        rp[j] = bm32 + 2 * ((int64_t)cand[has[j] ? rj : r] * W);
      }
      unsigned int x[kRowsInFlight][kCapW];
#pragma unroll
      for (int j = 0; j < kRowsInFlight; ++j)
#pragma unroll
        for (int k = 0; k < kCapW; ++k) x[j][k] = (k < Wc) ? rp[j][cw[k]] : 0u;
      uint64_t m[kRowsInFlight] = {0, 0, 0, 0};
#pragma unroll
      for (int k = 0; k < kCapW; ++k) {
        const bool ok = (vmask >> k) & 1u;
#pragma unroll
        for (int j = 0; j < kRowsInFlight; ++j) {
          const uint64_t b = __ballot(ok && ((x[j][k] >> cb[k]) & 1u));
          if (lane == k) m[j] = b;
        }
      }
      if (lane < Wc) {
#pragma unroll
        for (int j = 0; j < kRowsInFlight; ++j)
          if (has[j]) A[(r + j * kGreedyWaves) * kCapStride + lane] = m[j];
      }
    }
    if (tid < 16) {
      const int lo = tid * 64;
      Pc[tid] = (lo + 64 <= pc) ? ~0ull : (lo < pc ? ((1ull << (pc - lo)) - 1ull) : 0ull);
    }
    if (tid == 0) misc[0] = csize;
    __syncthreads();
    stamp(3);
    int pcnt = pc;
    while (pcnt > 0) {
      if (cannot_win(csize + pcnt)) {
        gave_up = true;
// ... 35 lines not shown
        }
      }
      bestk = blockN_max_u64<kGreedyWaves>(bestk, red64);
      csize = misc[0];
      int left = 0;
      for (int w = 0; w < Wc; ++w) left += __popcll(Pc[w]);
      __syncthreads();
      if (left > 0 && bestk) {
        const int bc = (int)(0xffffffffu - (unsigned int)(bestk & 0xffffffffu));
        if (tid == 0) {
          C[csize] = cand[bc];
          misc[0] = csize + 1;
        }
        ++csize;
        if (tid < Wc) Pc[tid] &= A[bc * kCapStride + tid];
        __syncthreads();
        pcnt = 0;
        for (int w = 0; w < Wc; ++w) pcnt += __popcll(Pc[w]);
      } else {
        pcnt = 0;
      }
    }
  }
  (void)gave_up;
  stamp(4);
  if (tid == 0) {
    st->start_size[sidx] = csize;
    atomicMax(&st->heu_best, csize);
  }
  return csize;
}

template <int kGreedyThreads>
__device__ __attribute__((noinline)) void closure_round(const uint64_t* __restrict__ bm, int W, const uint64_t* Pa,
                                                        uint64_t* Pb, const int* alist, int cnt, int csize, int tid) {
  constexpr int kLanesPerRow = 16, kRowsPerGroup = 4, kChunk = 5;
  constexpr int kRowsPerPass = kGreedyThreads / kLanesPerRow * kRowsPerGroup;
  const int gid = tid / kLanesPerRow, sub = tid % kLanesPerRow;
#pragma unroll 1
  for (int k0 = 0; k0 < cnt; k0 += kRowsPerPass) {
    int v[kRowsPerGroup], c[kRowsPerGroup];
    const uint64_t* row[kRowsPerGroup];
#pragma unroll
    for (int r = 0; r < kRowsPerGroup; ++r) {
      const int k = k0 + gid * kRowsPerGroup + r;
      v[r] = k < cnt ? alist[k] : -1;
      row[r] = bm + (int64_t)(v[r] < 0 ? 0 : v[r]) * W;
      c[r] = 0;
    }
#pragma unroll 1
    for (int x0 = 0; x0 < W; x0 += kLanesPerRow * kChunk) {
      uint64_t buf[kRowsPerGroup][kChunk];
#pragma unroll
      for (int r = 0; r < kRowsPerGroup; ++r)
#pragma unroll
        for (int u = 0; u < kChunk; ++u) {
          const int x = x0 + u * kLanesPerRow + sub;
          buf[r][u] = (x < W && v[r] >= 0) ? row[r][x] : 0ull;
        }
#pragma unroll
      for (int u = 0; u < kChunk; ++u) {
        const int x = x0 + u * kLanesPerRow + sub;
        const uint64_t pa = x < W ? Pa[x] : 0ull;
#pragma unroll
        for (int r = 0; r < kRowsPerGroup; ++r) c[r] += __popcll(buf[r][u] & pa);
      }
    }
#pragma unroll
    for (int r = 0; r < kRowsPerGroup; ++r) {
      int cc = c[r];
      cc += __shfl_xor(cc, 8, 64);
      cc += __shfl_xor(cc, 4, 64);
      cc += __shfl_xor(cc, 2, 64);
      cc += __shfl_xor(cc, 1, 64);
      if (v[r] >= 0 && sub == 0 && cc >= csize)
        atomicOr(reinterpret_cast<unsigned long long*>(&Pb[v[r] >> 6]), 1ull << (v[r] & 63));
    }
  }
}

// ... 193 lines not shown
        smaller += (slot[hi] & 0xffffu) < (key & 0xffffu) ? 1 : 0;
      fin_key[q] = key;
      fin_pos[q] = lo + smaller;
    }
  }
  __syncthreads();
#pragma unroll
  for (int q = 0; q < kCoreCap / kDegThreads; ++q)
    if (fin_pos[q] >= 0) keys[fin_pos[q]] = fin_key[q];
  __syncthreads();
  {
    uint32_t* kout = key_pool + (size_t)blockIdx.y * kCoreCap;
    for (int r = tid; r < m; r += kDegThreads) kout[r] = keys[r];
    if (tid == 0) {
      counters[blockIdx.y] = m;
      counters[batch + blockIdx.y] = t;
    }
  }
}

constexpr int kRowStageWords = 256;
__global__ __launch_bounds__(kDegThreads) void degree_closure_rows_kernel(
    const ProbDesc* __restrict__ descs, const uint64_t* __restrict__ bitmap,
    uint64_t* __restrict__ comp_pool ,
    const uint32_t* __restrict__ key_pool ,
    const int32_t* __restrict__ counters, int batch) {
  TAIL_WAVE_PRIO();
  constexpr int kRows = 4, kGrp = 8;
  __shared__ unsigned int keys[kCoreCap];
  __shared__ __attribute__((aligned(16))) uint64_t rowbuf[kDegThreads / 64][kRows][kRowStageWords];
  const int m = counters[blockIdx.y];
  if (m < 2) return;
  const ProbDesc d = descs[blockIdx.y];
  const int W = d.W, tid = threadIdx.x, lane = tid & 63, wave = tid >> 6;
  const uint64_t* bm = bitmap + d.bm_off;
  {
    const uint32_t* kin = key_pool + (size_t)blockIdx.y * kCoreCap;
    for (int r = tid; r < m; r += kDegThreads) keys[r] = kin[r];
  }
  __syncthreads();
  const int ng = (m + 63) >> 6;
  uint64_t* comp = comp_pool + (size_t)blockIdx.y * kCoreCap * kCoreWords;
  const bool staged = W <= kRowStageWords;
  {
    const int G = gridDim.x;
    const int per = (((m + G - 1) / G) + 15) & ~15;
    const int k0 = min(m, (int)blockIdx.x * per), k1 = min(m, k0 + per);
    const unsigned int* bm32 = reinterpret_cast<const unsigned int*>(bm);
    for (int rb = k0 + wave * kRows; rb < k1; rb += 4 * kRows) {
      const unsigned int* rp[kRows];
      int rtile[kRows];
      uint64_t myword[kRows];
#pragma unroll
      for (int r = 0; r < kRows; ++r) {
        const int rr = min(rb + r, k1 - 1);
        const int v = (int)(keys[rr] & 0xffffu);
        rp[r] = bm32 + 2 * ((int64_t)v * W);
        rtile[r] = v >> 6;
        myword[r] = 0;
      }
      if (staged) {
        uint64_t wv[kRows][kRowStageWords / 64];
#pragma unroll
        for (int r = 0; r < kRows; ++r)
#pragma unroll
          for (int u = 0; u < kRowStageWords / 64; ++u)
            wv[r][u] = (64 * u + lane < W && 64 * u + lane >= rtile[r]) ? reinterpret_cast<const uint64_t*>(rp[r])[64 * u + lane] : 0ull;
#pragma unroll
        for (int r = 0; r < kRows; ++r)
#pragma unroll
          for (int u = 0; u < kRowStageWords / 64; ++u)
            if (64 * u < W) rowbuf[wave][r][64 * u + lane] = wv[r][u];
        __builtin_amdgcn_fence(__ATOMIC_ACQ_REL, "wavefront");
      }
      const unsigned int* rowlds = reinterpret_cast<const unsigned int*>(&rowbuf[wave][0][0]);
      auto groups = [&](auto staged_tag) {
        constexpr bool STAGED = decltype(staged_tag)::value;
        for (int g0 = 0; g0 < ng; g0 += kGrp) {
          unsigned int x[kRows][kGrp];
          int cbit[kGrp], cdeg[kGrp];
#pragma unroll
          for (int q = 0; q < kGrp; ++q) {
            const int idx = 64 * (g0 + q) + lane;
            const unsigned int key = idx < m ? keys[idx] : 0u;
            const int c = (int)(key & 0xffffu);
            cdeg[q] = idx < m ? (int)(key >> 16) : -1;
            cbit[q] = c & 31;
#pragma unroll
            for (int r = 0; r < kRows; ++r)
              x[r][q] = (cdeg[q] >= 0 && (c >> 6) >= rtile[r]) ? (STAGED ? rowlds[r * 2 * kRowStageWords + (c >> 5)] : rp[r][c >> 5]) : 0u;
// ... 384 lines not shown
    if (gridDim.x >= kMaxStarts) break;
    const int W = d.W, tid = threadIdx.x;
    uint64_t* Pa = reinterpret_cast<uint64_t*>(smem);
    uint64_t* Pb = Pa + ((W + 1) & ~1);
    const uint64_t* bm = bitmap + d.bm_off;
    int cnt = 0;
    __syncthreads();
    for (int w = tid >> 6; w < W; w += kGreedyWaves) {
      const int v = w * 64 + (tid & 63);
      const uint64_t bits = __ballot(v < d.n && deg[d.pt_off + v] >= csize);
      if ((tid & 63) == 0) {
        Pa[w] = bits;
        cnt += __popcll(bits);
      }
    }
    cnt = blockN_sum_i<kGreedyWaves>(cnt, red_c);
    constexpr int kClosureCap = 4096;
    int* alist = reinterpret_cast<int*>(Pb + ((W + 1) & ~1));
    for (int round = 0; round < 8 && cnt > csize && cnt <= 2 * csize + 256 && cnt <= kClosureCap; ++round) {
      if (tid == 0) next_s = 0;
      for (int w = tid; w < W; w += kGreedyThreads) Pb[w] = 0;
      __syncthreads();
      for (int w = tid; w < W; w += kGreedyThreads) {
        uint64_t bits = Pa[w];
        if (bits) {
          int pos = atomicAdd(&next_s, __popcll(bits));
          while (bits) {
            alist[pos++] = w * 64 + __builtin_ctzll(bits);
            bits &= bits - 1;
          }
        }
      }
      __syncthreads();
      closure_round<kGreedyThreads>(bm, W, Pa, Pb, alist, cnt, csize, tid);
      __syncthreads();
      int c2 = 0;
      for (int w = tid; w < W; w += kGreedyThreads) {
        const uint64_t x = Pb[w];
        Pa[w] = x;
        c2 += __popcll(x);
      }
      c2 = blockN_sum_i<kGreedyWaves>(c2, red_c);
      if (c2 == cnt) break;
      cnt = c2;
    }
    if (threadIdx.x == 0) {
      int nx = kMaxStarts;
      if (cnt <= csize) {
        __hip_atomic_store(&st->heu_closed, 1, __ATOMIC_RELAXED, __HIP_MEMORY_SCOPE_AGENT);
      } else if (!__hip_atomic_load(&st->heu_closed, __ATOMIC_RELAXED, __HIP_MEMORY_SCOPE_AGENT)) {
        nx = atomicAdd(&st->next_start, 1);
      }
      next_s = nx;
    }
    __syncthreads();
    sidx = next_s;
    __syncthreads();
  }
  if ((int)gridDim.y >= batch) return;
  }
}

constexpr int kSmallMaxW = kSmallCap / 64;
constexpr int kSmallSlotWords = 2 + kSmallMaxW;

__device__ __forceinline__ uint64_t wave_uniform_u64(uint64_t v) {
  const unsigned int lo = __builtin_amdgcn_readfirstlane((unsigned int)v);
// ... 100 lines not shown
    }
    if (csize > mybest) {
      mybest = csize;
      mystart = s0;
      bestw = cw;
      if (lane == 0) {
        atomicMax(wg_best, csize);
        atomicMax(best_seen, csize);
      }
    }
  }
  *mybest_out = mybest;
  *mystart_out = mystart;
  *bestw_out = bestw;
}

__global__ __launch_bounds__(256) void greedy_small_kernel(const ProbDesc* __restrict__ descs,
                                                           const uint64_t* __restrict__ bitmap,
                                                           const int32_t* __restrict__ deg, ProbState* __restrict__ states,
                                                           unsigned long long* __restrict__ slots ,
                                                           int32_t* __restrict__ best_seen ) {
  TAIL_WAVE_PRIO();
  extern __shared__ __attribute__((aligned(16))) char smem[];
  __shared__ uint64_t alive[kSmallMaxW], nxt[kSmallMaxW], outb[kSmallMaxW];
  __shared__ unsigned short alist[kSmallCap];
  __shared__ int csum[256];
  __shared__ unsigned long long wkey[4];
  __shared__ uint64_t wbits[4][kSmallMaxW];
  __shared__ int wg_best, changed;
  const int p = blockIdx.y, G = gridDim.x;
  const ProbDesc d = descs[p];
  ProbState* st = states + p;
  unsigned long long* slot = slots + ((size_t)p * G + blockIdx.x) * kSmallSlotWords;
  const int n = d.n, W = d.W, tid = threadIdx.x, lane = tid & 63, wave = tid >> 6;
  if (n < 2 || n > kSmallCap || st->deg_closed) {
    if (tid == 0) slot[0] = 0ull;
    return;
  }
  const uint64_t* bm = bitmap + d.bm_off;
  const int32_t* dg = deg + d.pt_off;
  int lb0 = 0;
  for (int k = 0; k < kMaxStarts; ++k) lb0 = max(lb0, st->start_size[k]);
  for (int w = wave; w < kSmallMaxW; w += 4) {
    const int v = 64 * w + lane;
    const uint64_t bits = __ballot(v < n && dg[v] >= lb0);
    if (lane == 0) alive[w] = w < W ? bits : 0ull;
  }
  if (tid == 0) wg_best = 0;
  __syncthreads();
  for (int round = 0; round < 64; ++round) {
    if (tid < kSmallMaxW) nxt[tid] = alive[tid];
    if (tid == 0) changed = 0;
    __syncthreads();
    for (int v = tid; v < n; v += 256) {
      if (!((alive[v >> 6] >> (v & 63)) & 1ull)) continue;
      const uint64_t* row = bm + (int64_t)v * W;
      uint64_t rw[kSmallMaxW];
#pragma unroll
      for (int x = 0; x < kSmallMaxW; ++x) rw[x] = x < W ? row[x] : 0ull;
      int c = 0;
#pragma unroll
      for (int x = 0; x < kSmallMaxW; ++x) c += __popcll(rw[x] & alive[x]);
      if (c < lb0) {
        atomicAnd(reinterpret_cast<unsigned long long*>(&nxt[v >> 6]), ~(1ull << (v & 63)));
        changed = 1;
      }
    }
    __syncthreads();
    const int ch = changed;
    if (tid < kSmallMaxW) alive[tid] = nxt[tid];
    __syncthreads();
    if (!ch) break;
  }
  int m = 0;
  for (int w = 0; w < W; ++w) m += __popcll(alive[w]);
  if (m <= lb0) {
    if (tid == 0) slot[0] = 0ull;
    return;
  }
  list_bits_ascending(alive, W, alist, csum, tid);
  const int Wc = (m + 63) >> 6;
  const int WBc = Wc <= 4 ? 4 : (Wc <= 8 ? 8 : 12);
  const int Sc = WBc | 1;
  uint64_t* A = reinterpret_cast<uint64_t*>(smem);
  for (int i = tid; i < 64 * Wc * Sc; i += 256) A[i] = 0ull;
  __syncthreads();
  for (int i0 = wave * 4; i0 < m; i0 += 16) {
    uint64_t words[4][kSmallMaxW];
#pragma unroll
    for (int r = 0; r < 4; ++r) {
      const int i = min(i0 + r, m - 1);
      const uint64_t* row = bm + (int64_t)alist[i] * W;
#pragma unroll
      for (int g = 0; g < kSmallMaxW; ++g) {
        const int c = 64 * g + lane;
        const int vc = (g < Wc && c < m) ? alist[c] : -1;
        words[r][g] = vc >= 0 ? ((row[vc >> 6] >> (vc & 63)) & 1ull) : 0ull;
      }
    }
#pragma unroll
    for (int r = 0; r < 4; ++r)
#pragma unroll
      for (int g = 0; g < kSmallMaxW; ++g)
        if (i0 + r < m && g < Wc) {
          const uint64_t mask = __ballot(words[r][g] != 0ull);
          if (lane == 0) A[(i0 + r) * Sc + g] = mask;
        }
  }
  __syncthreads();
  int mybest = 0, mystart = -1;
  uint64_t bestw = 0ull;
  const int first = blockIdx.x * 4 + wave, stride = G * 4;
  if (WBc == 4) small_all_starts<4>(A, m, lb0, first, stride, &wg_best, best_seen + p, lane, &mybest, &mystart, &bestw);
  else if (WBc == 8) small_all_starts<8>(A, m, lb0, first, stride, &wg_best, best_seen + p, lane, &mybest, &mystart, &bestw);
  else small_all_starts<12>(A, m, lb0, first, stride, &wg_best, best_seen + p, lane, &mybest, &mystart, &bestw);
  if (lane == 0) wkey[wave] = mybest > 0 ? (((unsigned long long)mybest << 32) | (0xffffffffu - (unsigned int)alist[max(mystart, 0)])) : 0ull;
  if (lane < kSmallMaxW) wbits[wave][lane] = bestw;
  if (tid < kSmallMaxW) outb[tid] = 0ull;
  __syncthreads();
  unsigned long long kbest = 0;
  int wbest = 0;
  for (int k = 0; k < 4; ++k)
    if (wkey[k] > kbest) {
      kbest = wkey[k];
      wbest = k;
// ... 178 lines not shown
    hipLaunchKernelGGL(greedy_clique_kernel<256>, dim3(nblk, rows), dim3(256), lds, s, d_desc, d_bitmap,
                       d_deg, d_state, d_start_cliques, total_n, reinterpret_cast<long long*>(d_trace), batch);
  }
}

__global__ __launch_bounds__(256) void peel_round_kernel(const ProbDesc* __restrict__ descs,
                                                         const uint64_t* __restrict__ bitmap,
                                                         ProbState* __restrict__ states,
                                                         const uint64_t* __restrict__ cur_mask,
                                                         uint64_t* __restrict__ nxt_mask,
                                                         int32_t* __restrict__ next_count ,
                                                         int batch) {
  TAIL_WAVE_PRIO();
  __shared__ unsigned long long neww;
  __shared__ int is_last;
  const ProbDesc d = descs[blockIdx.y];
  ProbState* st = states + blockIdx.y;
  const uint64_t* cur = cur_mask + d.w_off;
  if (st->peel_done) {
    if (!st->proven)
      for (int tile = blockIdx.x * 256 + threadIdx.x; tile < d.W; tile += gridDim.x * 256) nxt_mask[d.w_off + tile] = cur[tile];
    return;
  }
  const int lane = threadIdx.x & 63, wave = threadIdx.x >> 6;
  for (int tile = blockIdx.x; tile < d.W; tile += gridDim.x) {
    const uint64_t aw = cur[tile];
    if (threadIdx.x == 0) neww = 0;
    __syncthreads();
    if (aw) {
      const int lb = st->lb;
      const uint64_t* bm = bitmap + d.bm_off;
      for (int r = wave; r < 64; r += 4) {
        if (!((aw >> r) & 1ull)) continue;
        const uint64_t* row = bm + (int64_t)(tile * 64 + r) * d.W;
        int c = 0;
        for (int w = lane; w < d.W; w += 64) c += __popcll(row[w] & cur[w]);
        c = wave_sum_i(c);
        if (lane == 0 && c >= lb) atomicOr(&neww, 1ull << r);
      }
    }
    __syncthreads();
    if (threadIdx.x == 0) {
      nxt_mask[d.w_off + tile] = neww;
      if (neww) atomicAdd(next_count + blockIdx.y, __popcll(neww));
    }
    __syncthreads();
  }
  if (threadIdx.x == 0) {
    __threadfence();
    is_last = atomicAdd(next_count + batch + blockIdx.y, 1) == (int)gridDim.x - 1;
  }
  __syncthreads();
  if (is_last && threadIdx.x == 0) {
    __threadfence();
    const int c = __hip_atomic_load(next_count + blockIdx.y, __ATOMIC_RELAXED, __HIP_MEMORY_SCOPE_AGENT);
    if (c == st->alive_count) st->peel_done = 1;
    st->alive_count = c;
    if (c <= st->lb) {
      st->proven = 1;
      st->peel_done = 1;
    }
    __hip_atomic_store(next_count + blockIdx.y, 0, __ATOMIC_RELAXED, __HIP_MEMORY_SCOPE_AGENT);
    __hip_atomic_store(next_count + batch + blockIdx.y, 0, __ATOMIC_RELAXED, __HIP_MEMORY_SCOPE_AGENT);
  }
}

void launch_select_best(hipStream_t s, const ProbDesc* d_desc, int batch, int max_W,
// ... 29 lines not shown
```

teaser-plusplus_amd/csrc/solver.hip:

```cpp
#include <algorithm>
#include <cmath>
#include <cstdio>
#include <cstdlib>
#include <cstring>
#include <atomic>
#include <chrono>
#include <condition_variable>
#include <deque>
#include <memory>
#include <mutex>
#include <string>
#include <thread>
#include <vector>

#include "host_common.h"
#include "internal.h"

namespace thip {
void launch_select_best(hipStream_t s, const ProbDesc* d_desc, int batch, int max_W,
                        const int32_t* d_deg, ProbState* d_state, const int32_t* d_start_cliques,
                        int64_t total_n, int32_t* d_clique, uint64_t* d_alive_a, int do_peel,
                        const void* d_small_slots = nullptr, int small_G = 0);
void launch_peel_rounds(hipStream_t s, const ProbDesc* d_desc, int batch, int max_W,
                        const uint64_t* d_bitmap, ProbState* d_state, uint64_t* d_alive_a,
// ... 221 lines not shown
struct LaneFinisher {
  std::thread th;
  std::mutex m;
  std::condition_variable cv;
  std::atomic<int> state{0};
  std::vector<teaser_solution_c> out;
  int32_t rc = TEASER_HIP_OK;
};

struct teaser_hip_solver : HandleBase {
  teaser_params_c params;
  teaser_params_c params_given;
  int profiling = 0;
  teaser_profile_c prof;
  std::vector<hipEvent_t> ev_pool;
  struct Span { int stage; hipEvent_t a, b; };
  std::vector<Span> spans;
  size_t ev_used = 0;

  int batch = 0;
  int max_n = 0, max_W = 0;
  int64_t total_n = 0, total_bm = 0, total_w = 0, total_tims = 0;
  std::vector<ProbDesc> descs;
  std::vector<ProbState> states;
  std::vector<int64_t> tim_off;
  std::vector<int32_t> exact_run;
  std::vector<int32_t> heu_size;
  std::vector<int32_t> prob_status;
  const double* cur_src = nullptr;
  const double* cur_dst = nullptr;
  bool have_graph = false;
  bool bm_lower_missing = false;

  SolverBuf d_desc, d_state, d_src, d_dst, d_bitmap, d_deg, d_clique, d_start_cliques, d_alive_a,
      d_alive_b, d_next_count, d_weights, d_rot_inl, d_trans_inl, d_tls_scratch, d_tim_off,
      d_pk, d_prep, d_work, d_core, d_small;
  SolverBuf c_sel, c_colour, c_tent, c_xlist, c_list_a, c_list_b, c_counts, c_bits, c_class, c_mis;
  std::vector<int32_t> colour_x;
  SolverBuf x_order, x_src, x_dst, x_bitmap, x_ctrl, x_clique, x_arena, x_probs, x_probs2, x_keys, x_xbits, x_tasks;
  SolverBuf s_a, s_b, s_c, s_d, s_e;
  teaser_hip_features* features = nullptr;

  PinnedBuf pin_states;
  PinnedBuf pin_in;
  PinnedBuf pin_pts;
  PinnedBuf pin_ep;
  bool spec_bounds_next = false;
  bool spec_mis_fits = true;
  int last_unproven = 0;
  bool skip_heuristic_next = false;
  int closure_open_prev = 0;
  int heu_blocks = 0;
  int heu_rows = 0;

  struct Pending {
    const double* d_src = nullptr;
    const double* d_dst = nullptr;
    int batch = 0, mode = 0;
    bool need_graph = false;
    bool spec_bounds = false;
    bool closure = false;
    bool heuristic_enqueued = true;
    int64_t total_n = 0, tls_stride = 0;
  } pend;
  std::vector<teaser_hip_solver*> lanes;
  std::vector<std::pair<int, int>> route;
// ... 689 lines not shown
  d.w_off = w_off;
  return d;
}

ProbState initial_state(int heu_blocks) {
  ProbState st;
  memset(&st, 0, sizeof(st));
  st.scale = 1.0;
  st.R[0] = st.R[4] = st.R[8] = 1.0;
  st.gnc_cost = INFINITY;
  st.next_start = heu_blocks;
  for (int k = 0; k < kMaxStarts; ++k) st.start_vertex[k] = -1;
  return st;
}

int32_t layout_batch(teaser_hip_solver* h, const int64_t* pt_off, const int32_t* n, int batch, bool closure) {
  h->batch = batch;
  h->descs.assign((size_t)batch, ProbDesc());
  h->tim_off.assign((size_t)batch, 0);
  h->exact_run.assign((size_t)batch, 0);
  h->heu_size.assign((size_t)batch, 0);
  h->prob_status.assign((size_t)batch, TEASER_HIP_OK);
  h->colour_x.assign((size_t)batch, -1);
  int max_n = 0;
  for (int b = 0; b < batch; ++b) max_n = std::max(max_n, n[b]);
  const bool closure_ahead = closure && max_n <= 65536;
  h->heu_blocks = heuristic_blocks_per_problem(batch, (max_n + 63) / 64, closure_ahead ? h->closure_open_prev : -1);
  h->heu_rows = closure_ahead && h->closure_open_prev * 4 <= batch ? std::min(batch, std::max(4, 2 * h->closure_open_prev)) : 0;
  h->states.assign((size_t)batch, initial_state(h->heu_blocks));
  int64_t bm = 0, wo = 0, tims = 0, maxpt = 0;
  for (int b = 0; b < batch; ++b) {
    if (n[b] < 0) return TEASER_HIP_ERR_BAD_ARG;
    const ProbDesc d = h->descs[(size_t)b] = problem_desc(n[b], pt_off[b], bm, wo);
    bm += (int64_t)d.n * d.W;
    wo += d.W;
    h->tim_off[(size_t)b] = tims;
    const int64_t kt = h->params.rotation_tim_graph == TEASER_TIM_CHAIN ? (int64_t)d.n : (int64_t)d.n * (d.n - 1) / 2;
    tims += kt + 2;
    maxpt = std::max<int64_t>(maxpt, d.pt_off + d.n);
  }
  h->max_n = max_n;
  h->max_W = (max_n + 63) / 64;
  h->total_n = maxpt;
  h->total_bm = bm;
  h->total_w = wo;
  h->total_tims = tims;
  return TEASER_HIP_OK;
}

int32_t solve_packed_enqueue(teaser_hip_solver* h, const double* d_src, const double* d_dst,
                             const int64_t* pt_off, const int32_t* n, int batch, bool fp64_k1) {
  hipStream_t s = h->stream;
  hipStream_t s1 = s;
  const teaser_params_c& P = h->params;
  if (!params_supported(P)) {
    h->err = "rotation_estimation_algorithm must be GNC_TLS, FGR or QUATRO";
    return TEASER_HIP_ERR_UNSUPPORTED;
  }
  const int mode = effective_mode(P);
  h->cur_src = d_src;
  h->cur_dst = d_dst;
  h->have_graph = false;
  h->pend.closure = false;
  h->pend.heuristic_enqueued = true;
  const int32_t lrc = layout_batch(h, pt_off, n, batch, mode == TEASER_INLIER_PMC_EXACT && setting(S_DEG_CLOSURE) != 0);
  if (lrc != TEASER_HIP_OK) return lrc;
  const int max_n = h->max_n;
// ... 938 lines not shown
  CHECK_PROBLEM(h, problem);
  if (!len) return TEASER_HIP_ERR_BAD_ARG;
  const ProbDesc& d = h->descs[(size_t)problem];
  const ProbState& st = h->states[(size_t)problem];
  const int64_t cnt = st.clique_size > 1 ? st.n_trans : 0;
  const int64_t cap = *len;
  *len = cnt;
  if (!buf) return TEASER_HIP_OK;
  if (cap < cnt) return TEASER_HIP_ERR_BAD_ARG;
  std::vector<int32_t> ti((size_t)cnt), cl((size_t)st.clique_size);
  if (cnt > 0) {
    HIPCHK(h, hipMemcpy(ti.data(), h->d_trans_inl.as<int32_t>() + d.pt_off, (size_t)cnt * 4, hipMemcpyDeviceToHost));
    HIPCHK(h, hipMemcpy(cl.data(), h->d_clique.as<int32_t>() + d.pt_off, (size_t)st.clique_size * 4, hipMemcpyDeviceToHost));
  }
  for (int64_t k = 0; k < cnt; ++k) buf[k] = cl[(size_t)ti[(size_t)k]];
  return TEASER_HIP_OK;
}

int32_t teaser_hip_get_inlier_graph_bitmap(teaser_hip_solver* h, int32_t problem, uint64_t* buf,
                                           int64_t* len) {
  CHECK_PROBLEM(h, problem);
  if (!h->have_graph) {
    if (len) *len = 0;
    return len ? TEASER_HIP_OK : TEASER_HIP_ERR_BAD_ARG;
  }
  const ProbDesc& d = h->descs[(size_t)problem];
  if (buf && h->bm_lower_missing) {
    launch_tim_graph_mfma(h->stream, kTimMirror, h->d_desc.as<ProbDesc>(), h->batch, h->max_n, 0, nullptr, nullptr, nullptr,
                          nullptr, nullptr, 0, h->d_bitmap.as<uint64_t>(), h->d_state.as<ProbState>(), nullptr, 0.0, 0.0);
    HIPCHK(h, hipGetLastError());
    HIPCHK(h, hipStreamSynchronize(h->stream));
    h->bm_lower_missing = false;
  }
  return copy_out(h, h->d_bitmap.as<uint64_t>() + d.bm_off, (int64_t)d.n * d.W, buf, len);
}

int32_t teaser_hip_get_degrees(teaser_hip_solver* h, int32_t problem, int32_t* buf, int64_t* len) {
  CHECK_PROBLEM(h, problem);
  if (!h->have_graph) {
    if (len) *len = 0;
    return len ? TEASER_HIP_OK : TEASER_HIP_ERR_BAD_ARG;
  }
  const ProbDesc& d = h->descs[(size_t)problem];
  return copy_out(h, h->d_deg.as<int32_t>() + d.pt_off, (int64_t)d.n, buf, len);
}

TEASER_HIP_API int32_t teaser_hip_probe_k1_worklist(teaser_hip_solver* h, uint64_t* regions, int64_t* stride_words,
                                                    int64_t* used_regions, int32_t* problems, uint32_t* seg_counts) {
  int32_t problem = 0;
  CHECK_PROBLEM(h, problem);
  if (!stride_words || !used_regions || !problems || !h->d_work.p || !h->d_prep.p) return TEASER_HIP_ERR_BAD_ARG;
  std::vector<int32_t> n((size_t)h->batch);
  int max_n = 0;
  for (int b = 0; b < h->batch; ++b) max_n = std::max(max_n, n[(size_t)b] = h->descs[(size_t)b].n);
  *problems = h->batch;
  HIPCHK(h, hipDeviceSynchronize());
  HIPCHK(h, (hipError_t)tim_probe_worklist(h->d_prep.p, h->d_work.p, tim_work_items(n.data(), h->batch), h->batch, max_n,
                                           reinterpret_cast<unsigned long long*>(regions), stride_words, used_regions,
                                           seg_counts));
  return TEASER_HIP_OK;
}

int32_t teaser_hip_solve_for_rotation(teaser_hip_solver* h, const double* src, const double* dst,
                                      int32_t k, double noise_bound, double* rotation,
                                      uint8_t* inlier_mask, double* cost, int32_t* iterations) {
  if (!h || !src || !dst || k <= 0 || !rotation) return TEASER_HIP_ERR_BAD_ARG;
  (void)hipSetDevice(h->device);
// ... 108 lines not shown
  if (m > ((int64_t)1 << 30)) {
    h->err = "solveForScale: at most 2^30 TIMs (as the reference)";
    return TEASER_HIP_ERR_UNSUPPORTED;
  }
  (void)hipSetDevice(h->device);
  hipStream_t s = h->stream;
  const double beta = 2 * h->params.noise_bound * std::sqrt(h->params.cbar2);
  HIPCHK(h, h->s_a.ensure((size_t)m * 24));
  HIPCHK(h, h->s_b.ensure((size_t)m * 24));
  HIPCHK(h, hipMemcpyAsync(h->s_a.p, v1, (size_t)m * 24, hipMemcpyHostToDevice, s));
  HIPCHK(h, hipMemcpyAsync(h->s_b.p, v2, (size_t)m * 24, hipMemcpyHostToDevice, s));
  *scale = 1.0;
  if (h->params.estimate_scaling) {
    HIPCHK(h, h->x_src.ensure((size_t)m * 8));
    HIPCHK(h, h->x_dst.ensure((size_t)m * 8));
    launch_tim_scale_terms(s, h->s_a.as<double>(), h->s_b.as<double>(), m, beta, 1, h->x_src.as<double>(),
                           h->x_dst.as<double>(), nullptr);
    return run_scalar_tls(h, h->x_src.as<double>(), h->x_dst.as<double>(), m, scale, inlier_mask);
  }
  HIPCHK(h, h->s_e.ensure((size_t)m + 16));
  launch_tim_scale_terms(s, h->s_a.as<double>(), h->s_b.as<double>(), m, beta, 0, nullptr, nullptr,
                         h->s_e.as<uint8_t>());
  HIPCHK(h, hipGetLastError());
  if (inlier_mask) HIPCHK(h, hipMemcpyAsync(inlier_mask, h->s_e.p, (size_t)m, hipMemcpyDeviceToHost, s));
  HIPCHK(h, hipStreamSynchronize(s));
  return TEASER_HIP_OK;
}

int32_t teaser_hip_max_clique(teaser_hip_solver* h, const uint64_t* bitmap, int32_t n,
                              int32_t* clique, int32_t* clique_size, int32_t* exact_run) {
  if (!h || !bitmap || n <= 0 || !clique || !clique_size) return TEASER_HIP_ERR_BAD_ARG;
  (void)hipSetDevice(h->device);
  hipStream_t s = h->stream;
  const int W = (n + 63) / 64;
  const int mode = effective_mode(h->params);
  if (mode == TEASER_INLIER_KCORE_HEU && n > 65536) {
    h->err = "KCORE_HEU supports at most 65536 vertices";
    return TEASER_HIP_ERR_UNSUPPORTED;
  }
  const int64_t off = 0;
  int32_t rc = layout_batch(h, &off, &n, 1, false);
  if (rc != TEASER_HIP_OK) return rc;
  h->batch = 0;
  h->pend.spec_bounds = false;
  h->bm_lower_missing = false;
  ProbState& st = h->states[0];
  HIPCHK(h, h->d_desc.ensure(sizeof(ProbDesc)));
  HIPCHK(h, h->d_state.ensure(sizeof(ProbState)));
  HIPCHK(h, h->d_bitmap.ensure((size_t)n * W * 8));
  HIPCHK(h, h->d_deg.ensure((size_t)n * 4));
  HIPCHK(h, h->d_clique.ensure((size_t)n * 4));
  HIPCHK(h, h->d_start_cliques.ensure((size_t)n * 4 * kMaxStarts));
  HIPCHK(h, h->d_alive_a.ensure((size_t)W * 8));
  HIPCHK(h, h->d_alive_b.ensure((size_t)W * 8));
  HIPCHK(h, h->d_next_count.ensure(32));
  HIPCHK(h, hipMemcpyAsync(h->d_desc.p, h->descs.data(), sizeof(ProbDesc), hipMemcpyHostToDevice, s));
  HIPCHK(h, hipMemcpyAsync(h->d_state.p, &st, sizeof(st), hipMemcpyHostToDevice, s));
  HIPCHK(h, hipMemcpyAsync(h->d_bitmap.p, bitmap, (size_t)n * W * 8, hipMemcpyHostToDevice, s));
  HIPCHK(h, hipMemsetAsync(h->d_next_count.p, 0, 32, s));
  const bool exact = (mode == TEASER_INLIER_PMC_EXACT);
  launch_degrees(s, h->d_desc.as<ProbDesc>(), 1, n, h->d_bitmap.as<uint64_t>(), h->d_deg.as<int32_t>(),
                 h->d_state.as<ProbState>());
  rc = enqueue_heuristic_stage(h, 1, mode, false);
  if (rc != TEASER_HIP_OK) return rc;
  if (mode == TEASER_INLIER_KCORE_HEU) {
    HIPCHK(h, h->c_colour.ensure(4 * (size_t)n));
    HIPCHK(h, h->c_tent.ensure(4 * (size_t)n));
    launch_kcore_heuristic(s, h->d_desc.as<ProbDesc>(), 1, h->d_bitmap.as<uint64_t>(), h->d_deg.as<int32_t>(),
                           h->d_state.as<ProbState>(), h->c_colour.as<int32_t>(), h->c_tent.as<int32_t>(),
                           h->d_clique.as<int32_t>(), h->params.kcore_heuristic_threshold);
  }
  HIPCHK(h, hipGetLastError());
  HIPCHK(h, hipMemcpyAsync(&st, h->d_state.p, sizeof(st), hipMemcpyDeviceToHost, s));
  HIPCHK(h, hipStreamSynchronize(s));
  if (exact && n >= 2) {
    bool changed = false;
    rc = close_clique_bounds(h, 1, n, &changed);
    if (rc != TEASER_HIP_OK) return rc;
  }
  if (exact_run) *exact_run = h->exact_run[0];
  *clique_size = st.clique_size;
  if (st.clique_size > 0)
    HIPCHK(h, hipMemcpy(clique, h->d_clique.p, (size_t)st.clique_size * 4, hipMemcpyDeviceToHost));
  return h->prob_status[0];
}

int32_t teaser_hip_submit_batch(teaser_hip_solver* h, const double* src, const double* dst,
                                const int64_t* point_offset, const int32_t* n, int32_t batch,
                                int32_t flags, int32_t* ticket) {
  if (!h || !ticket || batch <= 0 || !src || !dst || !point_offset || !n) return TEASER_HIP_ERR_BAD_ARG;
  if (batch > kMaxBatch) return over_batch_limit(h);
// ... 296 lines not shown
```

Baseline: 111,700.

## Pad adjacency bitmap rows to a multiple of eight words

Changes the inlier-graph bitmap layout so each row's stride is rounded up to a multiple of 8 uint64 words, and updates every graph, clique and heuristic kernel to index rows with the padded stride. The intent is aligned row starts for wide vector and buffer loads and stores, and fewer partial cache-line accesses. Padding words are zero-filled by the builders. Host paths that hand the bitmap in or out now repack rows, and a new API exposes the padded rows directly. The cost is extra memory and host-side copy loops for external bitmaps.

```diff
diff --git a/include/teaser_hip.h b/include/teaser_hip.h
--- a/include/teaser_hip.h
+++ b/include/teaser_hip.h
@@ -157,6 +157,8 @@
 TEASER_HIP_API int32_t teaser_hip_get_inlier_graph_bitmap(teaser_hip_solver* h, int32_t problem, uint64_t* buf,
                                            int64_t* len );
 TEASER_HIP_API int32_t teaser_hip_get_degrees(teaser_hip_solver* h, int32_t problem, int32_t* buf, int64_t* len);
+TEASER_HIP_API int32_t teaser_hip_get_inlier_graph_rows(teaser_hip_solver* h, int32_t problem, uint64_t* buf,
+                                         int64_t* len , int32_t* stride_words);
 
 TEASER_HIP_API int32_t teaser_hip_solve_for_rotation(teaser_hip_solver* h, const double* src, const double* dst,
                                       int32_t k, double noise_bound, double* rotation_rowmajor,
diff --git a/teaser-plusplus_amd/__init__.py b/teaser-plusplus_amd/__init__.py
--- a/teaser-plusplus_amd/__init__.py
+++ b/teaser-plusplus_amd/__init__.py
@@ -103,7 +103,7 @@
     "teaser_hip_solve_device", "teaser_hip_solve_correspondences", "teaser_hip_solve_batch",
     "teaser_hip_solve_batch_device", "teaser_hip_get_max_clique", "teaser_hip_get_rotation_inliers",
     "teaser_hip_get_translation_inliers", "teaser_hip_get_input_ordered_translation_inliers",
-    "teaser_hip_get_inlier_graph_bitmap", "teaser_hip_get_degrees", "teaser_hip_solve_for_rotation",
+    "teaser_hip_get_inlier_graph_bitmap", "teaser_hip_get_inlier_graph_rows", "teaser_hip_get_degrees", "teaser_hip_solve_for_rotation",
     "teaser_hip_solve_for_translation", "teaser_hip_scalar_tls", "teaser_hip_max_clique",
     "teaser_hip_set_profiling", "teaser_hip_set_option", "teaser_hip_get_option", "teaser_hip_get_profile", "teaser_hip_get_stream",
     "teaser_hip_last_error", "teaser_hip_abi_version", "teaser_hip_device_count", "teaser_hip_host_alloc",
@@ -215,6 +215,7 @@
                "teaser_hip_get_input_ordered_translation_inliers", "teaser_hip_get_degrees"):
         getattr(L, nm).argtypes = [_vp, C.c_int32, _ip, _i64p]
     L.teaser_hip_get_inlier_graph_bitmap.argtypes = [_vp, C.c_int32, _u64p, _i64p]
+    L.teaser_hip_get_inlier_graph_rows.argtypes = [_vp, C.c_int32, _u64p, _i64p, _ip]
     L.teaser_hip_solve_for_rotation.argtypes = [_vp, _dp, _dp, C.c_int32, C.c_double, _dp, _u8p, _dp, _ip]
     L.teaser_hip_solve_for_translation.argtypes = [_vp, _dp, _dp, C.c_int32, _dp, _u8p]
     L.teaser_hip_scalar_tls.argtypes = [_vp, _dp, _dp, C.c_int32, _dp, _u8p]
diff --git a/teaser-plusplus_amd/csrc/internal.h b/teaser-plusplus_amd/csrc/internal.h
--- a/teaser-plusplus_amd/csrc/internal.h
+++ b/teaser-plusplus_amd/csrc/internal.h
@@ -24,6 +24,7 @@
   int64_t bm_off;
   int64_t w_off;
 };
+constexpr int bm_stride(int W) { return (W + 7) & ~7; }
 
 #ifndef TEASER_TAIL_PRIO
 #define TEASER_TAIL_PRIO 3
diff --git a/teaser-plusplus_amd/csrc/kernels_clique.hip b/teaser-plusplus_amd/csrc/kernels_clique.hip
--- a/teaser-plusplus_amd/csrc/kernels_clique.hip
+++ b/teaser-plusplus_amd/csrc/kernels_clique.hip
@@ -917,7 +917,7 @@
     for (int k = wave; k < xc; k += 4) {
       const int x = xlist[d.pt_off + k];
       if (!((Xb[x >> 6] >> (x & 63)) & 1ull)) continue;
-      const uint64_t* row = bm + (int64_t)x * W;
+      const uint64_t* row = bm + (int64_t)x * bm_stride(W);
       for (int w = lane; w < W; w += 64) {
         const uint64_t v = row[w] & al[w];
         if (v) atomicOr(reinterpret_cast<unsigned long long*>(&Cb[w]), v);
@@ -1069,7 +1069,7 @@
   const int32_t* order = order_pool + pb.order_off;
   uint64_t* out = bitmap_pool + pb.bm_off;
   for (int i = blockIdx.x * 4 + wave; i < n2; i += gridDim.x * 4) {
-    const uint64_t* row = bitmap + d.bm_off + (int64_t)order[i] * d.W;
+    const uint64_t* row = bitmap + d.bm_off + (int64_t)order[i] * bm_stride(d.W);
     for (int wo = 0; wo < W2; ++wo) {
       const int j = wo * 64 + lane;
       bool e = false;
@@ -1310,7 +1310,7 @@
     const int v = list[d.pt_off + it];
     F[lane] = 0ull;
     __builtin_amdgcn_fence(__ATOMIC_ACQ_REL, "wavefront");
-    const uint64_t* row = bitmap + d.bm_off + (int64_t)v * d.W;
+    const uint64_t* row = bitmap + d.bm_off + (int64_t)v * bm_stride(d.W);
     for (int w0 = 0; w0 < d.W; w0 += 64 * kRowWordsPerLane) {
       uint64_t words[kRowWordsPerLane];
 #pragma unroll
@@ -1388,7 +1388,7 @@
     if (consider) {
       const int tv = tn[v];
       const unsigned int pv = colour_hash(v, round, 0xabcdef1u);
-      const uint64_t* row = bitmap + d.bm_off + (int64_t)v * d.W;
+      const uint64_t* row = bitmap + d.bm_off + (int64_t)v * bm_stride(d.W);
       for (int w0 = 0; w0 < d.W; w0 += 64 * kRowWordsPerLane) {
         uint64_t words[kRowWordsPerLane];
 #pragma unroll
@@ -1552,7 +1552,7 @@
       }
       F[lane] = 0ull;
       __builtin_amdgcn_fence(__ATOMIC_ACQ_REL, "wavefront");
-      const uint64_t* row = bitmap + d.bm_off + (int64_t)v * d.W;
+      const uint64_t* row = bitmap + d.bm_off + (int64_t)v * bm_stride(d.W);
       for (int w0 = 0; w0 < d.W; w0 += 64 * kRowWordsPerLane) {
         uint64_t words[kRowWordsPerLane];
 #pragma unroll
@@ -1631,7 +1631,7 @@
       if (tv >= 0) {
         const unsigned int mine = 0x8000u | (unsigned int)tv;
         const unsigned int pv = colour_hash(v, r, 0xabcdef1u);
-        const uint64_t* row = bitmap + d.bm_off + (int64_t)v * d.W;
+        const uint64_t* row = bitmap + d.bm_off + (int64_t)v * bm_stride(d.W);
         for (int w0 = 0; w0 < d.W; w0 += 64 * kRowWordsPerLane) {
           uint64_t words[kRowWordsPerLane];
 #pragma unroll
@@ -1748,7 +1748,7 @@
   for (int root = blockIdx.y; root < xc; root += gridDim.y) {
   const int x = xlist[d.pt_off + root];
   __syncthreads();
-  for (int w = threadIdx.x; w < d.W; w += 256) Rx[w] = bm[(int64_t)x * d.W + w] & al[w];
+  for (int w = threadIdx.x; w < d.W; w += 256) Rx[w] = bm[(int64_t)x * bm_stride(d.W) + w] & al[w];
   __syncthreads();
   int cnt = 0;
   for (int w = blockIdx.x * 4 + wave; w < d.W; w += 4 * gridDim.x) {
@@ -1759,8 +1759,8 @@
       const bool two = bits != 0ull;
       const int y1 = two ? w * 64 + __builtin_ctzll(bits) : y0;
       bits &= bits - (two ? 1ull : 0ull);
-      const uint64_t* r0 = bm + (int64_t)y0 * d.W;
-      const uint64_t* r1 = bm + (int64_t)y1 * d.W;
+      const uint64_t* r0 = bm + (int64_t)y0 * bm_stride(d.W);
+      const uint64_t* r1 = bm + (int64_t)y1 * bm_stride(d.W);
       int c0 = 0, c1 = 0;
       for (int k0 = 0; k0 < d.W; k0 += 64 * 8) {
         uint64_t a[8], b[8];
@@ -1896,7 +1896,7 @@
   uint64_t* nc = mb.nc + (size_t)blockIdx.y * mb.cap * mb.max_W;
   const uint64_t* bm = bitmap + d.bm_off;
   for (int c = blockIdx.x; c < lbc; c += gridDim.x) {
-    const uint64_t* row = bm + (int64_t)cl[c] * d.W;
+    const uint64_t* row = bm + (int64_t)cl[c] * bm_stride(d.W);
     for (int w = threadIdx.x; w < d.W; w += 256) nc[(size_t)c * mb.max_W + w] = row[w];
   }
 }
@@ -2099,7 +2099,7 @@
       static_assert(kMisBatch <= 64 && kTpc * kPpt == kMisBatch && kPpt % kGrp == 0, "thread mapping of the adjacency gather");
       const int a = t / kTpc;
       const int ua = a < ncand ? cand[a] : 0;
-      const uint64_t* rowa = bm + (int64_t)ua * W;
+      const uint64_t* rowa = bm + (int64_t)ua * bm_stride(W);
       unsigned long long bits = 0ull;
 #pragma unroll
       for (int g0 = 0; g0 < kPpt; g0 += kGrp) {
@@ -2136,7 +2136,7 @@
 #pragma unroll
       for (int q = 0; q < kFly; ++q) {
         if (todo) {
-          rows[q] = bm + (int64_t)cand[__builtin_ctzll(todo)] * W;
+          rows[q] = bm + (int64_t)cand[__builtin_ctzll(todo)] * bm_stride(W);
           todo &= todo - 1ull;
         } else {
           rows[q] = nullptr;
@@ -2211,7 +2211,7 @@
     const int cv = col[v];
     if (cv < 0) continue;
     int bad = 0;
-    const uint64_t* row = bitmap + d.bm_off + (int64_t)v * d.W;
+    const uint64_t* row = bitmap + d.bm_off + (int64_t)v * bm_stride(d.W);
     for (int w = lane; w < d.W; w += 64) {
       uint64_t bits = row[w];
       while (bits) {
@@ -2462,7 +2462,7 @@
         const int b = __builtin_ctzll(f);
         f &= f - 1;
         if ((ord++ & (kCoreWaves - 1)) != wave) continue;
-        const uint64_t* row = bm + (int64_t)(w * 64 + b) * W;
+        const uint64_t* row = bm + (int64_t)(w * 64 + b) * bm_stride(W);
         for (int x = lane; x < W; x += 64) {
           uint64_t m = row[x] & alive[x];
           while (m) {
diff --git a/teaser-plusplus_amd/csrc/kernels_graph.hip b/teaser-plusplus_amd/csrc/kernels_graph.hip
--- a/teaser-plusplus_amd/csrc/kernels_graph.hip
+++ b/teaser-plusplus_amd/csrc/kernels_graph.hip
@@ -126,7 +126,7 @@
                                               const double* __restrict__ pd,
                                               uint64_t* __restrict__ bm, int n, int W, int I,
                                               int Jbase, const EdgeConst& kc, double* cbw) {
-  const int T = W;
+  const int T = W, S = bm_stride(W);
   const int lane = threadIdx.x & 63;
   const int i = I * 64 + lane;
   const bool vi = i < n;
@@ -174,10 +174,12 @@
     const uint64_t colmask = (n - j0 >= 64) ? ~0ull : ((1ull << (n - j0)) - 1ull);
     own &= colmask;
     if (J == I) own &= ~(1ull << lane);
-    if (vi) bm[(int64_t)i * W + J] = own;
+    if (vi) bm[(int64_t)i * S + J] = own;
     if (J != I && j0 + lane < n) {
-      bm[(int64_t)(j0 + lane) * W + I] = trw & rowmask;
-    }
+      bm[(int64_t)(j0 + lane) * S + I] = trw & rowmask;
+    }
+    if (J == T - 1 && vi)
+      for (int w = T; w < S; ++w) bm[(int64_t)i * S + w] = 0ull;
   }
 }
 
@@ -502,7 +504,7 @@
     ProbState* __restrict__ states, int32_t* __restrict__ deg, unsigned long long* __restrict__ regions, int Tmax) {
   const ProbDesc d = descs[blockIdx.y];
   const int n = d.n, W = d.W;
-  const int T = W;
+  const int T = W, S = bm_stride(W);
   int Ig, X;
   fxr::decode_block((int)blockIdx.x, (int)gridDim.x, gyr, CHUNKS, &Ig, &X);
   constexpr int kBlockColTiles = kMfmaColTiles * CHUNKS;
@@ -578,7 +580,7 @@
   const __amdgpu_buffer_rsrc_t deg_rsrc = __builtin_amdgcn_make_buffer_rsrc(
       (void*)(deg + d.pt_off), 0, (int)((unsigned int)n * 4u), 0x00020000);
   const __amdgpu_buffer_rsrc_t bm_rsrc = __builtin_amdgcn_make_buffer_rsrc(
-      (void*)bm, 0, (int)((unsigned int)n * (unsigned int)W * 8u), 0x00020000);
+      (void*)bm, 0, (int)((unsigned int)n * (unsigned int)S * 8u), 0x00020000);
   int degacc = 0;
   const int cq = c - 4 * h;
   const int selfq = (cq >= 0 && (cq & 4) == 0) ? ((cq & 3) | ((cq >> 3) << 2)) : -1;
@@ -790,7 +792,7 @@
         const uint4 lo = *reinterpret_cast<const uint4*>(&lds_tr[Jr][r][0]);
         const uint4 hi = *reinterpret_cast<const uint4*>(&lds_tr[Jr][r][2]);
         const bool rowok = J < Jc1 && j < n;
-        const unsigned int base = ((unsigned int)j * (unsigned int)W + (unsigned int)I0) * 8u;
+        const unsigned int base = ((unsigned int)j * (unsigned int)S + (unsigned int)I0) * 8u;
         if (Jc0 > I0 + 3 && I0 + 3 < T) {
           const int cnt = (__builtin_popcount(lo.x) + __builtin_popcount(lo.y)) + (__builtin_popcount(lo.z) + __builtin_popcount(lo.w)) +
                           (__builtin_popcount(hi.x) + __builtin_popcount(hi.y)) + (__builtin_popcount(hi.z) + __builtin_popcount(hi.w));
@@ -821,14 +823,14 @@
     }
     if (nact > 0) {
       const int kk = lane & 7, J = Jc0 + kk;
-      const bool colok = J >= Ja && J < Jc1;
-      const unsigned int off0 = ((unsigned int)(I * 64 + (lane >> 3)) * (unsigned int)W + (unsigned int)J) * 8u;
+      const bool pad = J >= T, colok = (J >= Ja && J < Jc1) || pad;
+      const unsigned int off0 = ((unsigned int)(I * 64 + (lane >> 3)) * (unsigned int)S + (unsigned int)J) * 8u;
 #pragma unroll
       for (int it = 0; it < 8; ++it) {
         const int r = it * 8 + (lane >> 3);
-        const uint64_t w = lds_own[wave][r][kk];
+        const uint64_t w = pad ? 0ull : lds_own[wave][r][kk];
         __builtin_amdgcn_raw_buffer_store_b64(u32x2{(unsigned int)w, (unsigned int)(w >> 32)}, bm_rsrc,
-                                              (colok && I * 64 + r < n) ? off0 + (unsigned int)it * 64u * (unsigned int)W : kOobOffset,
+                                              (colok && I * 64 + r < n) ? off0 + (unsigned int)it * 64u * (unsigned int)S : kOobOffset,
                                               0, 0);
       }
     }
@@ -911,9 +913,9 @@
   const TimPrep tpr = prep[prob];
   const unsigned int cap = tpr.seg_cap;
   const ProbDesc d = descs[prob];
-  const int n = d.n, W = d.W;
+  const int n = d.n, W = d.W, S = bm_stride(W);
   if (total > cap) {
-    const int64_t words = (int64_t)n * W;
+    const int64_t words = (int64_t)n * S;
     uint64_t* bm = bitmap + d.bm_off;
     for (int64_t w = (int64_t)blockIdx.x * 256 + threadIdx.x; w < words; w += (int64_t)gridDim.x * 256) bm[w] = 0;
     if (blockIdx.x == 0 && threadIdx.x == 0) states[prob].k1_overflow = 1;
@@ -924,7 +926,7 @@
     const uint64_t* bm = bitmap + d.bm_off;
     const int lane = threadIdx.x & 63;
     for (int row = blockIdx.x * 4 + (threadIdx.x >> 6); row < n; row += gridDim.x * 4) {
-      const uint64_t* r = bm + (int64_t)row * W;
+      const uint64_t* r = bm + (int64_t)row * S;
       int c = 0;
       for (int w = lane; w < W; w += 64) c += __popcll(r[w]);
       c = wave_sum_i(c);
@@ -963,7 +965,7 @@
       cx = ps[3 * col]; cy = ps[3 * col + 1]; cz = ps[3 * col + 2];
       ex = pd[3 * col]; ey = pd[3 * col + 1]; ez = pd[3 * col + 2];
     }
-    unsigned int* wp = bm32 + 2 * ((int64_t)r * W + (col >> 6)) + ((col >> 5) & 1);
+    unsigned int* wp = bm32 + 2 * ((int64_t)r * S + (col >> 6)) + ((col >> 5) & 1);
     const unsigned int bit = 1u << (col & 31);
     bool prov;
     if (STAGED && (r >> 6) != (col >> 6)) {
@@ -980,7 +982,7 @@
     atomicXor(wp, bit);
     atomicAdd(dg + r, e ? 1 : -1);
     if ((r >> 6) != (col >> 6)) {
-      if (!upper) atomicXor(bm32 + 2 * ((int64_t)col * W + (r >> 6)) + ((r >> 5) & 1), 1u << (r & 31));
+      if (!upper) atomicXor(bm32 + 2 * ((int64_t)col * S + (r >> 6)) + ((r >> 5) & 1), 1u << (r & 31));
       atomicAdd(dg + col, e ? 1 : -1);
     }
   };
@@ -1050,7 +1052,7 @@
                                                                uint64_t* __restrict__ bitmap,
                                                                const ProbState* __restrict__ states, int skip_closed) {
   const ProbDesc d = descs[blockIdx.y];
-  const int n = d.n, W = d.W, T = W;
+  const int n = d.n, W = d.W, T = W, S = bm_stride(W);
   if (T < 2 || (skip_closed && states[blockIdx.y].deg_closed)) return;
   const int lane = threadIdx.x & 63;
   const int runs = (T + kMirrorRun - 1) / kMirrorRun;
@@ -1063,7 +1065,7 @@
     for (int k = 0; k < kMirrorRun; ++k) {
       out[k] = 0ull;
       if (Ia + k >= Ib) continue;
-      const uint64_t x = bm[(int64_t)(64 * (Ia + k) + lane) * W + J];
+      const uint64_t x = bm[(int64_t)(64 * (Ia + k) + lane) * S + J];
 #pragma unroll
       for (int c = 0; c < 64; ++c) {
         const uint64_t m = __builtin_amdgcn_ballot_w64(((x >> c) & 1ull) != 0ull);
@@ -1074,7 +1076,7 @@
     if (row < n) {
 #pragma unroll
       for (int k = 0; k < kMirrorRun; ++k)
-        if (Ia + k < Ib) bm[(int64_t)row * W + Ia + k] = out[k];
+        if (Ia + k < Ib) bm[(int64_t)row * S + Ia + k] = out[k];
     }
   }
 }
@@ -1255,7 +1257,7 @@
   const ProbDesc d = descs[blockIdx.y];
   const int lane = threadIdx.x & 63;
   for (int row = blockIdx.x * 4 + (threadIdx.x >> 6); row < d.n; row += gridDim.x * 4) {
-    const uint64_t* r = bitmap + d.bm_off + (int64_t)row * d.W;
+    const uint64_t* r = bitmap + d.bm_off + (int64_t)row * bm_stride(d.W);
     int c = 0;
     for (int w = lane; w < d.W; w += 64) c += __popcll(r[w]);
     c = wave_sum_i(c);
diff --git a/teaser-plusplus_amd/csrc/kernels_heuristic.hip b/teaser-plusplus_amd/csrc/kernels_heuristic.hip
--- a/teaser-plusplus_amd/csrc/kernels_heuristic.hip
+++ b/teaser-plusplus_amd/csrc/kernels_heuristic.hip
@@ -55,7 +55,7 @@
   if (tr && threadIdx.x == 0) tr[6] = tr[7] = 0;
   stamp(0);
   const ProbDesc d = descs[prob];
-  const int n = d.n, W = d.W;
+  const int n = d.n, W = d.W, S = bm_stride(W);
   const int Wpad = (W + 1) & ~1;
   uint64_t* P = reinterpret_cast<uint64_t*>(smem);
   uint64_t* U = P + Wpad;
@@ -107,7 +107,7 @@
   if (tid == 0) C[0] = v0;
   int pc = 0;
   for (int w = tid; w < W; w += kGreedyThreads) {
-    const uint64_t x = bm[(int64_t)v0 * W + w];
+    const uint64_t x = bm[(int64_t)v0 * S + w];
     P[w] = x;
     pc += __popcll(x);
   }
@@ -148,7 +148,7 @@
       int c = 0;
       __syncthreads();
       for (int w = tid; w < W; w += kGreedyThreads) {
-        const uint64_t x = P[w] & bm[(int64_t)u * W + w];
+        const uint64_t x = P[w] & bm[(int64_t)u * S + w];
         P[w] = x;
         c += __popcll(x);
       }
@@ -218,7 +218,7 @@
         for (int q = 0; q < kStreamRows; ++q) {
           on[q] = i0 + q < pc;
           vv[q] = clist[on[q] ? i0 + q : i0];
-          rr[q] = bm + (int64_t)vv[q] * W;
+          rr[q] = bm + (int64_t)vv[q] * S;
         }
         int cc[kStreamRows];
 #pragma unroll
@@ -268,8 +268,8 @@
         const bool two = bits != 0ull;
         const int b1 = two ? __builtin_ctzll(bits) : b0;
         bits &= bits - (two ? 1ull : 0ull);
-        const uint64_t* r0 = bm + (int64_t)(w * 64 + b0) * W;
-        const uint64_t* r1 = bm + (int64_t)(w * 64 + b1) * W;
+        const uint64_t* r0 = bm + (int64_t)(w * 64 + b0) * S;
+        const uint64_t* r1 = bm + (int64_t)(w * 64 + b1) * S;
         int c0 = 0, c1 = 0;
         for (int x0 = 0; x0 < W; x0 += 64 * 8) {
           uint64_t ra[8], rb[8];
@@ -333,7 +333,7 @@
       ++csize;
       int c = 0;
       for (int w = tid; w < W; w += kGreedyThreads) {
-        const uint64_t x = P[w] & bm[(int64_t)u * W + w];
+        const uint64_t x = P[w] & bm[(int64_t)u * S + w];
         P[w] = x;
         c += __popcll(x);
       }
@@ -407,7 +407,7 @@
       for (int j = 0; j < kRowsInFlight; ++j) {
         const int rj = r + j * kGreedyWaves;
         has[j] = rj < pc;
-        rp[j] = bm32 + 2 * ((int64_t)cand[has[j] ? rj : r] * W);
+        rp[j] = bm32 + 2 * ((int64_t)cand[has[j] ? rj : r] * S);
       }
       unsigned int x[kRowsInFlight][kCapW];
 #pragma unroll
@@ -509,7 +509,7 @@
 }
 
 template <int kGreedyThreads>
-__device__ __attribute__((noinline)) void closure_round(const uint64_t* __restrict__ bm, int W, const uint64_t* Pa,
+__device__ __attribute__((noinline)) void closure_round(const uint64_t* __restrict__ bm, int W, int S , const uint64_t* Pa,
                                                         uint64_t* Pb, const int* alist, int cnt, int csize, int tid) {
   constexpr int kLanesPerRow = 16, kRowsPerGroup = 4, kChunk = 5;
   constexpr int kRowsPerPass = kGreedyThreads / kLanesPerRow * kRowsPerGroup;
@@ -522,7 +522,7 @@
     for (int r = 0; r < kRowsPerGroup; ++r) {
       const int k = k0 + gid * kRowsPerGroup + r;
       v[r] = k < cnt ? alist[k] : -1;
-      row[r] = bm + (int64_t)(v[r] < 0 ? 0 : v[r]) * W;
+      row[r] = bm + (int64_t)(v[r] < 0 ? 0 : v[r]) * S;
       c[r] = 0;
     }
 #pragma unroll 1
@@ -782,7 +782,7 @@
   const int m = counters[blockIdx.y];
   if (m < 2) return;
   const ProbDesc d = descs[blockIdx.y];
-  const int W = d.W, tid = threadIdx.x, lane = tid & 63, wave = tid >> 6;
+  const int W = d.W, S = bm_stride(W), tid = threadIdx.x, lane = tid & 63, wave = tid >> 6;
   const uint64_t* bm = bitmap + d.bm_off;
   {
     const uint32_t* kin = key_pool + (size_t)blockIdx.y * kCoreCap;
@@ -805,7 +805,7 @@
       for (int r = 0; r < kRows; ++r) {
         const int rr = min(rb + r, k1 - 1);
         const int v = (int)(keys[rr] & 0xffffu);
-        rp[r] = bm32 + 2 * ((int64_t)v * W);
+        rp[r] = bm32 + 2 * ((int64_t)v * S);
         rtile[r] = v >> 6;
         myword[r] = 0;
       }
@@ -1256,7 +1256,7 @@
         }
       }
       __syncthreads();
-      closure_round<kGreedyThreads>(bm, W, Pa, Pb, alist, cnt, csize, tid);
+      closure_round<kGreedyThreads>(bm, W, bm_stride(W), Pa, Pb, alist, cnt, csize, tid);
       __syncthreads();
       int c2 = 0;
       for (int w = tid; w < W; w += kGreedyThreads) {
@@ -1423,7 +1423,7 @@
   const ProbDesc d = descs[p];
   ProbState* st = states + p;
   unsigned long long* slot = slots + ((size_t)p * G + blockIdx.x) * kSmallSlotWords;
-  const int n = d.n, W = d.W, tid = threadIdx.x, lane = tid & 63, wave = tid >> 6;
+  const int n = d.n, W = d.W, S = bm_stride(W), tid = threadIdx.x, lane = tid & 63, wave = tid >> 6;
   if (n < 2 || n > kSmallCap || st->deg_closed) {
     if (tid == 0) slot[0] = 0ull;
     return;
@@ -1445,7 +1445,7 @@
     __syncthreads();
     for (int v = tid; v < n; v += 256) {
       if (!((alive[v >> 6] >> (v & 63)) & 1ull)) continue;
-      const uint64_t* row = bm + (int64_t)v * W;
+      const uint64_t* row = bm + (int64_t)v * S;
       uint64_t rw[kSmallMaxW];
 #pragma unroll
       for (int x = 0; x < kSmallMaxW; ++x) rw[x] = x < W ? row[x] : 0ull;
@@ -1481,7 +1481,7 @@
 #pragma unroll
     for (int r = 0; r < 4; ++r) {
       const int i = min(i0 + r, m - 1);
-      const uint64_t* row = bm + (int64_t)alist[i] * W;
+      const uint64_t* row = bm + (int64_t)alist[i] * S;
 #pragma unroll
       for (int g = 0; g < kSmallMaxW; ++g) {
         const int c = 64 * g + lane;
@@ -1726,7 +1726,7 @@
       const uint64_t* bm = bitmap + d.bm_off;
       for (int r = wave; r < 64; r += 4) {
         if (!((aw >> r) & 1ull)) continue;
-        const uint64_t* row = bm + (int64_t)(tile * 64 + r) * d.W;
+        const uint64_t* row = bm + (int64_t)(tile * 64 + r) * bm_stride(d.W);
         int c = 0;
         for (int w = lane; w < d.W; w += 64) c += __popcll(row[w] & cur[w]);
         c = wave_sum_i(c);
diff --git a/teaser-plusplus_amd/csrc/solver.hip b/teaser-plusplus_amd/csrc/solver.hip
--- a/teaser-plusplus_amd/csrc/solver.hip
+++ b/teaser-plusplus_amd/csrc/solver.hip
@@ -277,6 +277,7 @@
   bool have_graph = false;
   bool bm_lower_missing = false;
 
+  std::vector<uint64_t> bm_stage;
   SolverBuf d_desc, d_state, d_src, d_dst, d_bitmap, d_deg, d_clique, d_start_cliques, d_alive_a,
       d_alive_b, d_next_count, d_weights, d_rot_inl, d_trans_inl, d_tls_scratch, d_tim_off,
       d_pk, d_prep, d_work, d_core, d_small;
@@ -1032,7 +1033,7 @@
   for (int b = 0; b < batch; ++b) {
     if (n[b] < 0) return TEASER_HIP_ERR_BAD_ARG;
     const ProbDesc d = h->descs[(size_t)b] = problem_desc(n[b], pt_off[b], bm, wo);
-    bm += (int64_t)d.n * d.W;
+    bm += (int64_t)d.n * bm_stride(d.W);
     wo += d.W;
     h->tim_off[(size_t)b] = tims;
     const int64_t kt = h->params.rotation_tim_graph == TEASER_TIM_CHAIN ? (int64_t)d.n : (int64_t)d.n * (d.n - 1) / 2;
@@ -2037,7 +2038,37 @@
     HIPCHK(h, hipStreamSynchronize(h->stream));
     h->bm_lower_missing = false;
   }
-  return copy_out(h, h->d_bitmap.as<uint64_t>() + d.bm_off, (int64_t)d.n * d.W, buf, len);
+  if (!len) return TEASER_HIP_ERR_BAD_ARG;
+  const int64_t cap = *len, count = (int64_t)d.n * d.W;
+  *len = count;
+  if (!buf) return TEASER_HIP_OK;
+  if (cap < count) return TEASER_HIP_ERR_BAD_ARG;
+  const int S = bm_stride(d.W);
+  const uint64_t* rows = h->d_bitmap.as<uint64_t>() + d.bm_off;
+  if (S == d.W) {
+    if (count > 0) HIPCHK(h, hipMemcpy(buf, rows, (size_t)count * 8, hipMemcpyDeviceToHost));
+    return TEASER_HIP_OK;
+  }
+  const int64_t blk = std::max<int64_t>(1, ((int64_t)4 << 20) / S);
+  std::vector<uint64_t> stage((size_t)(std::min<int64_t>(blk, d.n) * S));
+  for (int64_t r0 = 0; r0 < d.n; r0 += blk) {
+    const int64_t nr = std::min<int64_t>(blk, d.n - r0);
+    HIPCHK(h, hipMemcpy(stage.data(), rows + r0 * S, (size_t)(nr * S) * 8, hipMemcpyDeviceToHost));
+    for (int64_t r = 0; r < nr; ++r) memcpy(buf + (r0 + r) * d.W, stage.data() + r * S, (size_t)d.W * 8);
+  }
+  return TEASER_HIP_OK;
+}
+
+int32_t teaser_hip_get_inlier_graph_rows(teaser_hip_solver* h, int32_t problem, uint64_t* buf, int64_t* len,
+                                         int32_t* stride_words) {
+  CHECK_PROBLEM(h, problem);
+  const ProbDesc& d = h->descs[(size_t)problem];
+  if (stride_words) *stride_words = bm_stride(d.W);
+  if (!h->have_graph) {
+    if (len) *len = 0;
+    return len ? TEASER_HIP_OK : TEASER_HIP_ERR_BAD_ARG;
+  }
+  return copy_out(h, h->d_bitmap.as<uint64_t>() + d.bm_off, (int64_t)d.n * bm_stride(d.W), buf, len);
 }
 
 int32_t teaser_hip_get_degrees(teaser_hip_solver* h, int32_t problem, int32_t* buf, int64_t* len) {
@@ -2212,7 +2243,7 @@
   if (!h || !bitmap || n <= 0 || !clique || !clique_size) return TEASER_HIP_ERR_BAD_ARG;
   (void)hipSetDevice(h->device);
   hipStream_t s = h->stream;
-  const int W = (n + 63) / 64;
+  const int W = (n + 63) / 64, S = bm_stride(W);
   const int mode = effective_mode(h->params);
   if (mode == TEASER_INLIER_KCORE_HEU && n > 65536) {
     h->err = "KCORE_HEU supports at most 65536 vertices";
@@ -2227,7 +2258,7 @@
   ProbState& st = h->states[0];
   HIPCHK(h, h->d_desc.ensure(sizeof(ProbDesc)));
   HIPCHK(h, h->d_state.ensure(sizeof(ProbState)));
-  HIPCHK(h, h->d_bitmap.ensure((size_t)n * W * 8));
+  HIPCHK(h, h->d_bitmap.ensure((size_t)n * S * 8));
   HIPCHK(h, h->d_deg.ensure((size_t)n * 4));
   HIPCHK(h, h->d_clique.ensure((size_t)n * 4));
   HIPCHK(h, h->d_start_cliques.ensure((size_t)n * 4 * kMaxStarts));
@@ -2236,7 +2267,13 @@
   HIPCHK(h, h->d_next_count.ensure(32));
   HIPCHK(h, hipMemcpyAsync(h->d_desc.p, h->descs.data(), sizeof(ProbDesc), hipMemcpyHostToDevice, s));
   HIPCHK(h, hipMemcpyAsync(h->d_state.p, &st, sizeof(st), hipMemcpyHostToDevice, s));
-  HIPCHK(h, hipMemcpyAsync(h->d_bitmap.p, bitmap, (size_t)n * W * 8, hipMemcpyHostToDevice, s));
+  const uint64_t* up = bitmap;
+  if (S != W) {
+    h->bm_stage.assign((size_t)n * S, 0ull);
+    for (int64_t r = 0; r < n; ++r) memcpy(h->bm_stage.data() + r * S, bitmap + r * W, (size_t)W * 8);
+    up = h->bm_stage.data();
+  }
+  HIPCHK(h, hipMemcpyAsync(h->d_bitmap.p, up, (size_t)n * S * 8, hipMemcpyHostToDevice, s));
   HIPCHK(h, hipMemsetAsync(h->d_next_count.p, 0, 32, s));
   const bool exact = (mode == TEASER_INLIER_PMC_EXACT);
   launch_degrees(s, h->d_desc.as<ProbDesc>(), 1, n, h->d_bitmap.as<uint64_t>(), h->d_deg.as<int32_t>(),
```

After: 116,700, median of 6. 4.6% higher.
